# rockcarry/ffcnn

Measured on AMD Instinct MI355X. Metric: frames/sec yolo-fastest-1.1 @320x320 batch-64 per GPU (u8 BGR frames -> net_input's conversion in the first kernel -> full forward: conv stack + YOLO decode + NMS, boxes on rank 0), higher is better.
Workload: dtype f32

## Files before the change

ffcnn_amd/capi.py:

```python
import ctypes as C
import os
import subprocess

import numpy as np

HERE = os.path.dirname(os.path.abspath(__file__))
ROOT = os.path.dirname(HERE)
DATA = os.path.join(ROOT, "data")
CFG = os.path.join(DATA, "yolo-fastest-1.1.cfg")
WEIGHTS = os.path.join(DATA, "yolo-fastest-1.1.weights")

f32p = C.POINTER(C.c_float)


class FFGPU:
    MAX_DET = 128
    MERGE_LDS_SLOTS = 1024
    KEEP_ALL, COMPAT_V6, NO_GRAPH, NO_FUSE, HOST_DETS, SPLIT2, CONCURRENT, BF16_PW = 1, 2, 4, 8, 16, 32, 64, 128
    FEAT_FLAT, FEAT_MEAN, FEAT_MAX = 0, 1, 2
    POST_NONE, POST_SOFTMAX, POST_L2 = 0, 1, 2
    TOPK_MAX = 16
    RELABEL_KEEP_SCORE, RELABEL_LABEL_SCORE = 0, 1
    RELABEL_ENTRIES, RELABEL_MERGED = 0, 1
    K_AUTO, K_GENERIC, K_DW_STREAM, K_DW_LDS, K_PW_MFMA, K_PW_GEMM, _K6, K_DENSE_SMALL, K_IGEMM, K_PW_BF16, K_GROUP_THIN, K_PW_X3, K_CONV_X3, K_PW_X3T = range(14)
# ... 98 lines not shown
class Zone(C.Structure):
    _fields_ = [("x", C.c_float * 8), ("y", C.c_float * 8), ("nverts", C.c_int), ("dwell_frames", C.c_int), ("classes", C.c_uint * 4), ("reserved", C.c_int * 2)]


class Line(C.Structure):
    _fields_ = [("ax", C.c_float), ("ay", C.c_float), ("bx", C.c_float), ("by", C.c_float), ("classes", C.c_uint * 4)]


class Scene(C.Structure):
    _fields_ = [("zone", Zone * 8), ("line", Line * 8), ("nzones", C.c_int), ("nlines", C.c_int), ("anchor", C.c_int), ("reserved", C.c_int)]


class ZonesSpec(C.Structure):
    _fields_ = [("capacity", C.c_int), ("max_missed", C.c_int), ("identity", C.c_int), ("flags", C.c_int), ("min_score", C.c_float),
                ("gate_zone", C.c_uint), ("gate_line", C.c_uint), ("reserved", C.c_int)]


class ZoneSlot(C.Structure):
    _fields_ = [("id", C.c_int), ("px", C.c_float), ("py", C.c_float), ("inside", C.c_int), ("last", C.c_int), ("reserved", C.c_int * 3), ("since", C.c_int * 8)]


class TextItem(C.Structure):
    _fields_ = [("x", C.c_int), ("y", C.c_int), ("fg", C.c_ubyte * 4), ("bg", C.c_ubyte * 4), ("scale", C.c_ubyte), ("flags", C.c_ubyte), ("len", C.c_ubyte),
                ("reserved", C.c_ubyte), ("text", C.c_ubyte * 44)]


class CaptionSpec(C.Structure):
    _fields_ = [("min_score", C.c_float), ("flags", C.c_int), ("identity", C.c_int), ("scale", C.c_int), ("fg", C.c_ubyte * 4), ("color", C.c_ubyte * 4),
                ("palette", C.c_void_p), ("npalette", C.c_int), ("nnames", C.c_int), ("d_names", C.c_void_p)]


class SegItem(C.Structure):
    _fields_ = [("x0", C.c_int), ("y0", C.c_int), ("x1", C.c_int), ("y1", C.c_int), ("color", C.c_ubyte * 4), ("thickness", C.c_ubyte), ("dash", C.c_ubyte),
                ("flags", C.c_ubyte), ("reserved", C.c_ubyte), ("reserved2", C.c_int * 2)]


class OutlineSpec(C.Structure):
    _fields_ = [("flags", C.c_int), ("thickness", C.c_int), ("line_dash", C.c_int), ("marker", C.c_int), ("color", C.c_ubyte * 4), ("alarm", C.c_ubyte * 4),
                ("palette", C.c_void_p), ("npalette", C.c_int), ("reserved", C.c_int)]


class TrailPoint(C.Structure):
    _fields_ = [("x", C.c_int), ("y", C.c_int), ("frame", C.c_int)]


class TrailSlot(C.Structure):
    _fields_ = [("id", C.c_int), ("last", C.c_int), ("n", C.c_int), ("head", C.c_int), ("cx", C.c_int), ("cy", C.c_int), ("reserved", C.c_int * 2),
                ("ring", TrailPoint * 32)]


class TrailsSpec(C.Structure):
    _fields_ = [("capacity", C.c_int), ("max_missed", C.c_int), ("identity", C.c_int), ("flags", C.c_int), ("min_score", C.c_float), ("anchor", C.c_int),
                ("points", C.c_int), ("min_move", C.c_int), ("thickness", C.c_int), ("coast_dash", C.c_int), ("color", C.c_ubyte * 4), ("reserved0", C.c_int),
                ("palette", C.c_void_p), ("npalette", C.c_int), ("reserved", C.c_int)]


class HeatSpec(C.Structure):
    _fields_ = [("gw", C.c_int), ("gh", C.c_int), ("cell_log2", C.c_int), ("mode", C.c_int), ("flags", C.c_int), ("anchor", C.c_int), ("spread", C.c_int),
                ("gain", C.c_int), ("decay_shift", C.c_int), ("min_score", C.c_float), ("classes", C.c_void_p), ("nclasses", C.c_int), ("reserved", C.c_int)]


class HeatBlendSpec(C.Structure):
    _fields_ = [("gw", C.c_int), ("gh", C.c_int), ("cell_log2", C.c_int), ("full_scale", C.c_int), ("floor", C.c_int), ("opacity", C.c_int),
                ("sampling", C.c_int), ("flags", C.c_int), ("palette", C.c_void_p), ("reserved", C.c_int * 2)]


class MotionSpec(C.Structure):
    _fields_ = [("w", C.c_int), ("h", C.c_int), ("cell_log2", C.c_int), ("threshold", C.c_int), ("learn_shift", C.c_int), ("learn_shift_changed", C.c_int),
                ("min_pixels", C.c_int), ("cover", C.c_int), ("warmup", C.c_int), ("flags", C.c_int), ("min_score", C.c_float), ("nclasses", C.c_int),
                ("classes", C.c_void_p), ("reserved", C.c_int * 2)]


MOTION_DETS, MOTION_ROW, MOTION_WORDS, MOTION_MAX_SIDE = 128, 16, 8, 8192
MOTION_GATE_INVERT = 1
MOTION_ENTRIES, MOTION_MERGED = 0, 1
MOTION_ROW_HEADER = ("frame", "changed", "active", "x0", "y0", "x1", "y1", "warm")
MOTION_WORDS_HEADER = ("considered", "dropped", "outside", "moving", "warm", "frames")
MOTION_STATE_HEADER = 16
HEAT_MAX, HEAT_DETS, HEAT_ROW = 2 ** 31 - 1, 128, 8
HEAT_ANCHOR, HEAT_BOX = 0, 1
HEAT_NEAREST, HEAT_SMOOTH = 0, 1
HEAT_RAMP_ALPHA = 1
HEAT_ENTRIES, HEAT_MERGED = 0, 1
HEAT_ROW_HEADER = ("considered", "dropped", "outside", "frame", "peak", "saturated")
HEAT_STATE_HEADER = 16
TRAIL_POINTS, TRAILS_DETS, TRAILS_ROW = 32, 128, 16
TRAILS_COAST, TRAILS_TAPER = 1, 2
TRAILS_ENTRIES, TRAILS_MERGED = 0, 1
TRAILS_ROW_HEADER = ("considered", "known", "fresh", "refused", "duplicate", "anonymous", "dropped", "freed", "live", "frame", "appended", "drawn", "clipped")
TRAILS_STATE_HEADER = 16
SEG_ITEMS, SEG_LIMIT, OUTLINE_FIXED = 512, 1 << 20, 80
OUTLINE_ZONES, OUTLINE_LINES, OUTLINE_TICKS, OUTLINE_MARKERS, OUTLINE_ALARM = 1, 2, 4, 8, 16
TEXT_MAX, TEXT_ITEMS, TEXT_OPAQUE = 44, 256, 1
CAPTION_DETS = 128
CAPTION_NAME, CAPTION_SCORE, CAPTION_ID, CAPTION_OPAQUE = 1, 2, 4, 8
CAPTION_ENTRIES, CAPTION_MERGED = 0, 1
SCENE_ZONES, SCENE_LINES, ZONE_VERTS, ZONES_DETS, ZONES_ROW = 8, 8, 8, 128, 64
ZONES_NONE, ZONES_TYPE, ZONES_IDS = 0, 1, 2
ZONES_GATE_INVERT = 1
ZONES_ENTRIES, ZONES_MERGED = 0, 1
ZONES_EVENTS_HEADER = ("considered", "known", "fresh", "refused", "duplicate", "anonymous", "dropped", "freed", "live", "frame")
ZONES_STATE_HEADER = 144
TRACK_DETS = 128
TRACK_ENTRIES, TRACK_MERGED = 0, 1
TRACK_IDS_HEADER = ("considered", "matched", "born", "refused", "dropped", "freed", "live", "frame")
CROP_F32, CROP_U8 = 0, 1
CROP_ENTRIES, CROP_MERGED = 0, 1
REDACT_FILL, REDACT_MOSAIC = 0, 1
REDACT_OUTSIDE = 1
REDACT_ENTRIES, REDACT_MERGED = 0, 1
BLUR_OUTSIDE = 1
BLUR_ENTRIES, BLUR_MERGED = 0, 1
DRAW_ENTRIES, DRAW_MERGED = 0, 1
YUV_BT601_LIMITED, YUV_BT601_FULL, YUV_BT709_LIMITED, YUV_BT709_FULL = 0, 1, 2, 3

assert C.sizeof(LAYER) == 120 and C.sizeof(NET) == 104 and C.sizeof(BBOX) == 24
assert C.sizeof(FrameDets) == 16 + 24 * FFGPU.MAX_DET
assert C.sizeof(BgrFrame) == 24 and C.sizeof(Nv12Frame) == 40 and C.sizeof(Tile) == 16 and C.sizeof(TileRect) == 16
assert C.sizeof(DrawStyle) == 24 and C.sizeof(CropSpec) == 72 and C.sizeof(Crop) == 48
assert C.sizeof(TrackSpec) == 32 and C.sizeof(Track) == 48
assert C.sizeof(FeatureSpec) == 16 and C.sizeof(Label) == 8 and C.sizeof(RelabelSpec) == 16
assert C.sizeof(Gallery) == 40 and C.sizeof(RedactSpec) == 40 and C.sizeof(BlurSpec) == 40
assert C.sizeof(TextItem) == 64 and C.sizeof(CaptionSpec) == 48
assert C.sizeof(SegItem) == 32 and C.sizeof(OutlineSpec) == 40
assert C.sizeof(TrailPoint) == 12 and C.sizeof(TrailSlot) == 416 and C.sizeof(TrailsSpec) == 64
assert C.sizeof(HeatSpec) == 56 and C.sizeof(HeatBlendSpec) == 48
assert C.sizeof(MotionSpec) == 64
assert C.sizeof(Zone) == 96 and C.sizeof(Line) == 32 and C.sizeof(Scene) == 1040 and C.sizeof(ZonesSpec) == 32 and C.sizeof(ZoneSlot) == 64

BOX_DTYPE = np.dtype([("type", "<i4"), ("score", "<f4"), ("x1", "<f4"), ("y1", "<f4"), ("x2", "<f4"), ("y2", "<f4")])
DETS_DTYPE = np.dtype([("count", "<i4"), ("ncand", "<i4"), ("overflow", "<i4"), ("nfull", "<i4"),
                       ("box", BOX_DTYPE, (FFGPU.MAX_DET,))])
CROP_DTYPE = np.dtype([("target", "<i4"), ("box", "<i4"), ("type", "<i4"), ("score", "<f4"), ("x0", "<i4"), ("y0", "<i4"), ("w", "<i4"), ("h", "<i4"),
                       ("sw", "<i4"), ("sh", "<i4"), ("s1", "<i4"), ("s2", "<i4")])
TRACK_DTYPE = np.dtype([("id", "<i4"), ("type", "<i4"), ("score", "<f4"), ("x1", "<f4"), ("y1", "<f4"), ("x2", "<f4"), ("y2", "<f4"),
                        ("hits", "<i4"), ("missed", "<i4"), ("born", "<i4"), ("det", "<i4"), ("reserved", "<i4")])
ZONE_SLOT_DTYPE = np.dtype([("id", "<i4"), ("px", "<f4"), ("py", "<f4"), ("inside", "<i4"), ("last", "<i4"), ("reserved", "<i4", (3,)), ("since", "<i4", (8,))])
TRAIL_POINT_DTYPE = np.dtype([("x", "<i4"), ("y", "<i4"), ("frame", "<i4")])
TRAIL_SLOT_DTYPE = np.dtype([("id", "<i4"), ("last", "<i4"), ("n", "<i4"), ("head", "<i4"), ("cx", "<i4"), ("cy", "<i4"), ("reserved", "<i4", (2,)),
                             ("ring", TRAIL_POINT_DTYPE, (32,))])
LABEL_DTYPE = np.dtype([("index", "<i4"), ("value", "<f4")])
TEXT_ITEM_DTYPE = np.dtype([("x", "<i4"), ("y", "<i4"), ("fg", "u1", (4,)), ("bg", "u1", (4,)), ("scale", "u1"), ("flags", "u1"), ("len", "u1"), ("reserved", "u1"),
                            ("text", "u1", (44,))])
SEG_ITEM_DTYPE = np.dtype([("x0", "<i4"), ("y0", "<i4"), ("x1", "<i4"), ("y1", "<i4"), ("color", "u1", (4,)), ("thickness", "u1"), ("dash", "u1"), ("flags", "u1"),
                           ("reserved", "u1"), ("reserved2", "<i4", (2,))])

EXPORTS = ["net_load", "net_free", "net_input", "net_forward", "net_dump", "net_profile", "groupconv",
           "ffgpu_device_count", "ffgpu_set_device", "ffgpu_last_error", "ffgpu_build_info",
           "ffgpu_net_weights_dev", "ffgpu_net_weights_commit",
           "ffgpu_exec_create", "ffgpu_exec_destroy", "ffgpu_exec_batch", "ffgpu_exec_arena_bytes",
           "ffgpu_exec_kernel_count", "ffgpu_exec_work_model", "ffgpu_exec_set_scale", "ffgpu_exec_forward_dev", "ffgpu_exec_forward_host",
           "ffgpu_exec_forward_bgr_dev", "ffgpu_exec_forward_bgr_frames_dev", "ffgpu_exec_forward_nv12_frames_dev", "ffgpu_exec_dets_dev", "ffgpu_exec_dets_host", "ffgpu_exec_set_ring", "ffgpu_exec_set_ring_strided", "ffgpu_exec_read_dets", "ffgpu_exec_read_layer", "ffgpu_exec_hash_layers",
           "ffgpu_exec_read_boxes", "ffgpu_exec_cand_capacity", "ffgpu_exec_graph_captures",
           "ffgpu_exec_profile", "ffgpu_exec_profile_steps", "ffgpu_exec_step_model", "ffgpu_groupconv_dev", "ffgpu_groupconv_kernel_name", "ffgpu_groupconv_time_dev", "ffgpu_irb_dev", "ffgpu_irb_plan_text", "ffgpu_irb_stage_plan_text", "ffgpu_front_plan_text", "ffgpu_irb_instantiations", "ffgpu_knobs_text", "ffgpu_dwpw_dev", "ffgpu_packed_records_bytes", "ffgpu_pack_records", "ffgpu_unpack_records",
           "ffgpu_shard_range", "ffgpu_node_create", "ffgpu_node_destroy", "ffgpu_node_ndev", "ffgpu_node_shard", "ffgpu_node_set_scale",
           "ffgpu_node_input_dev", "ffgpu_node_input_slot_dev", "ffgpu_node_depth", "ffgpu_node_rccl_ranks", "ffgpu_node_forward", "ffgpu_node_forward_host",
           "ffgpu_node_submit", "ffgpu_node_wait", "ffgpu_node_run",
           "ffgpu_merge_tiles_scratch_bytes", "ffgpu_merge_tiles_dev", "ffgpu_exec_merge_tiles", "ffgpu_exec_merged_dev", "ffgpu_exec_read_merged",
           "ffgpu_exec_read_merged_boxes", "ffgpu_tile_plan",
           "ffgpu_draw_boxes_bgr_dev", "ffgpu_draw_boxes_nv12_dev", "ffgpu_exec_draw_bgr", "ffgpu_exec_draw_nv12",
           "ffgpu_crop_table_bytes", "ffgpu_crop_slot_bytes", "ffgpu_crop_boxes_bgr_dev", "ffgpu_crop_boxes_nv12_dev", "ffgpu_exec_crop_bgr", "ffgpu_exec_crop_nv12",
           "ffgpu_crops_to_source_dev",
           "ffgpu_track_state_bytes", "ffgpu_track_reset_dev", "ffgpu_track_boxes_dev", "ffgpu_exec_track",
           "ffgpu_feature_dim", "ffgpu_exec_feature_dim", "ffgpu_features_dev", "ffgpu_exec_features", "ffgpu_topk_dev", "ffgpu_crops_relabel_dev",
           "ffgpu_exec_relabel",
           "ffgpu_match_workspace_bytes", "ffgpu_match_dev", "ffgpu_gallery_enroll_dev",
           "ffgpu_redact_boxes_bgr_dev", "ffgpu_redact_boxes_nv12_dev", "ffgpu_exec_redact_bgr", "ffgpu_exec_redact_nv12",
           "ffgpu_blur_boxes_bgr_dev", "ffgpu_blur_boxes_nv12_dev", "ffgpu_exec_blur_bgr", "ffgpu_exec_blur_nv12",
           "ffgpu_zones_state_bytes", "ffgpu_scene_check", "ffgpu_zones_reset_dev", "ffgpu_zones_boxes_dev", "ffgpu_exec_zones",
           "ffgpu_font_builtin", "ffgpu_draw_text_bgr_dev", "ffgpu_draw_text_nv12_dev", "ffgpu_caption_boxes_dev", "ffgpu_exec_caption_bgr", "ffgpu_exec_caption_nv12",
           "ffgpu_caption_scene_dev",
           "ffgpu_draw_segments_bgr_dev", "ffgpu_draw_segments_nv12_dev", "ffgpu_outline_spec_check", "ffgpu_outline_scene_dev",
           "ffgpu_trails_state_bytes", "ffgpu_trails_spec_check", "ffgpu_trails_reset_dev", "ffgpu_trails_boxes_dev", "ffgpu_exec_trails",
           "ffgpu_heat_state_bytes", "ffgpu_heat_spec_check", "ffgpu_heat_blend_spec_check", "ffgpu_heat_palette", "ffgpu_heat_reset_dev", "ffgpu_heat_boxes_dev",
           "ffgpu_exec_heat", "ffgpu_heat_blend_bgr_dev", "ffgpu_heat_blend_nv12_dev",
           "ffgpu_motion_state_bytes", "ffgpu_motion_spec_check", "ffgpu_motion_reset_dev", "ffgpu_motion_update_bgr_dev", "ffgpu_motion_update_nv12_dev",
           "ffgpu_motion_gate_dev", "ffgpu_exec_motion_gate"]
DIAG_EXPORTS = ["ffgpu_membench", "ffgpu_pipe_probe", "ffgpu_pipe_probe2", "ffgpu_pipe_probe3", "ffgpu_mfma_floor", "ffgpu_diag_x3_term", "ffgpu_diag_xl_op", "ffgpu_clock_probe"]


def library_path():
    return os.environ.get("FFCNN_HIP_LIB") or os.path.join(HERE, "lib", "libffcnn_hip.so")


def build_library(force=False):
    cmd = ["make", "-C", os.path.join(HERE, "csrc")]
    if force:
        subprocess.check_call(cmd + ["clean"], stdout=subprocess.DEVNULL)
    subprocess.check_call(cmd, stdout=subprocess.DEVNULL)
    return library_path()


_lib = None


def lib():
    global _lib
    if _lib is not None:
        return _lib
    path = library_path()
    if not os.path.exists(path):
        raise RuntimeError("%s is missing: run `python -c 'import __graft_entry__ as g; g.build()'` "
                           "(the HIP extension is the only compute path)" % path)
    L = C.CDLL(path)
    vp, i, sz = C.c_void_p, C.c_int, C.c_size_t
    L.net_load.restype = C.POINTER(NET)
    L.net_load.argtypes = [C.c_char_p, C.c_char_p, i, i]
    L.net_free.argtypes = [C.POINTER(NET)]
    L.net_input.argtypes = [C.POINTER(NET), vp, i, i, f32p, f32p]
    L.net_forward.argtypes = [C.POINTER(NET)]
    L.net_dump.argtypes = [C.POINTER(NET)]
    L.net_profile.argtypes = [C.POINTER(NET)]
    L.groupconv.argtypes = [f32p, f32p, f32p] + [i] * 12 + [C.POINTER(f32p), C.POINTER(i)]
    L.ffgpu_last_error.restype = C.c_char_p
    L.ffgpu_build_info.restype = C.c_char_p
    if b" DIAG " in L.ffgpu_build_info() and os.environ.get("FFCNN_HIP_ALLOW_DIAG") != "1":
        raise RuntimeError("%s is a DIAG (lab) build of libffcnn_hip; set FFCNN_HIP_ALLOW_DIAG=1 to load it on purpose" % path)
    L.ffgpu_set_device.argtypes = [i]
    L.ffgpu_net_weights_dev.argtypes = [C.POINTER(NET), C.POINTER(vp), C.POINTER(sz)]
    L.ffgpu_net_weights_commit.argtypes = [C.POINTER(NET), vp]
    L.ffgpu_exec_create.restype = vp
    L.ffgpu_exec_create.argtypes = [C.POINTER(NET), i, i]
    L.ffgpu_exec_destroy.argtypes = [vp]
    L.ffgpu_exec_batch.argtypes = [vp]
    L.ffgpu_exec_arena_bytes.restype = sz
    L.ffgpu_exec_arena_bytes.argtypes = [vp]
    L.ffgpu_exec_kernel_count.argtypes = [vp]
    L.ffgpu_exec_work_model.argtypes = [vp, C.POINTER(C.c_double), C.POINTER(C.c_double)]
    L.ffgpu_exec_set_scale.argtypes = [vp, i, i]
    L.ffgpu_exec_forward_dev.argtypes = [vp, vp, vp]
    L.ffgpu_exec_forward_host.argtypes = [vp, f32p]
    L.ffgpu_exec_forward_bgr_dev.argtypes = [vp, vp, i, i, f32p, f32p, vp]
    L.ffgpu_exec_forward_bgr_frames_dev.argtypes = [vp, C.POINTER(BgrFrame), i, f32p, f32p, vp]
    L.ffgpu_exec_forward_nv12_frames_dev.argtypes = [vp, C.POINTER(Nv12Frame), i, f32p, f32p, vp]
    L.ffgpu_exec_dets_dev.argtypes = [vp, C.POINTER(vp), C.POINTER(sz)]
    L.ffgpu_exec_dets_host.restype = vp; L.ffgpu_exec_dets_host.argtypes = [vp]
    L.ffgpu_exec_set_ring.argtypes = [vp, vp, C.c_int]
    L.ffgpu_exec_set_ring_strided.argtypes = [vp, vp, C.c_int, C.c_int]
    L.ffgpu_exec_read_dets.argtypes = [vp, vp, i]
    L.ffgpu_exec_read_layer.argtypes = [vp, i, i, f32p, sz]
    L.ffgpu_exec_hash_layers.argtypes = [vp, vp, i]
    L.ffgpu_exec_profile.argtypes = [vp, vp, f32p]
    L.ffgpu_exec_profile_steps.argtypes = [vp, vp, C.POINTER(i), f32p, i]
    L.ffgpu_exec_step_model.argtypes = [vp, C.POINTER(i), C.POINTER(C.c_double), i]
    L.ffgpu_groupconv_dev.argtypes = [vp, vp, vp] + [i] * 15 + [vp]
    L.ffgpu_groupconv_kernel_name.restype = C.c_char_p
    L.ffgpu_groupconv_kernel_name.argtypes = [i] * 10
    L.ffgpu_groupconv_time_dev.restype = C.c_float
    L.ffgpu_groupconv_time_dev.argtypes = [vp, vp, vp] + [i] * 17 + [vp]
    L.ffgpu_irb_dev.restype = C.c_float
    L.ffgpu_irb_dev.argtypes = [vp] * 6 + [i] * 13 + [vp]
    L.ffgpu_irb_plan_text.argtypes = [i] * 12 + [C.c_char_p, i]
    L.ffgpu_irb_stage_plan_text.argtypes = [i] * 7 + [C.c_char_p, i]
    L.ffgpu_front_plan_text.argtypes = [i] * 4 + [C.c_char_p, i]
    L.ffgpu_irb_instantiations.argtypes = [C.c_char_p, i]
    L.ffgpu_knobs_text.argtypes = [C.c_char_p, i]
    L.ffgpu_exec_read_boxes.argtypes = [vp, i, vp, i]
    L.ffgpu_exec_cand_capacity.argtypes = [vp]
    L.ffgpu_exec_graph_captures.argtypes = [vp]
    L.ffgpu_dwpw_dev.restype = C.c_float
    L.ffgpu_dwpw_dev.argtypes = [vp] * 4 + [i] * 10 + [vp]
    L.ffgpu_packed_records_bytes.restype = C.c_size_t
    L.ffgpu_packed_records_bytes.argtypes = [i, i]
    L.ffgpu_pack_records.restype = i
    L.ffgpu_pack_records.argtypes = [vp, i, C.c_long, i, i, vp, vp]
    L.ffgpu_shard_range.argtypes = [i, i, i, C.POINTER(i), C.POINTER(i)]
    L.ffgpu_shard_range.restype = None
    L.ffgpu_node_create.restype = vp
    L.ffgpu_node_create.argtypes = [C.POINTER(NET), i, C.POINTER(i), i, i, i]
    L.ffgpu_node_destroy.argtypes = [vp]
    L.ffgpu_node_ndev.argtypes = [vp]
    L.ffgpu_node_shard.argtypes = [vp, i, C.POINTER(i), C.POINTER(i), C.POINTER(i)]
    L.ffgpu_node_set_scale.argtypes = [vp, i, i]
    L.ffgpu_node_input_dev.restype = vp
    L.ffgpu_node_input_dev.argtypes = [vp, i]
    L.ffgpu_node_input_slot_dev.restype = vp
    L.ffgpu_node_input_slot_dev.argtypes = [vp, i, i]
    L.ffgpu_node_depth.argtypes = [vp]
    if hasattr(L, "ffgpu_node_rccl_ranks"):
        L.ffgpu_node_rccl_ranks.argtypes = [vp]
    L.ffgpu_node_submit.restype = C.c_long
    L.ffgpu_node_submit.argtypes = [vp, f32p]
    L.ffgpu_node_wait.argtypes = [vp, C.c_long, vp]
    L.ffgpu_node_run.argtypes = [vp, C.c_long, vp]
    L.ffgpu_unpack_records.argtypes = [vp, i, i, vp]
    L.ffgpu_node_forward.argtypes = [vp, vp]
    L.ffgpu_node_forward_host.argtypes = [vp, f32p, vp]
    L.ffgpu_merge_tiles_scratch_bytes.restype = sz
    L.ffgpu_merge_tiles_scratch_bytes.argtypes = [i, i]
    L.ffgpu_merge_tiles_dev.argtypes = [vp, vp, i, C.POINTER(Tile), i, i, C.c_float, i, vp, vp, vp, sz, vp]
    L.ffgpu_exec_merge_tiles.argtypes = [vp, C.POINTER(Tile), i, i, vp]
    L.ffgpu_exec_merged_dev.argtypes = [vp, C.POINTER(vp), C.POINTER(sz)]
    L.ffgpu_exec_read_merged.argtypes = [vp, vp, i]
    L.ffgpu_exec_read_merged_boxes.argtypes = [vp, i, vp, i]
    L.ffgpu_tile_plan.argtypes = [i] * 7 + [C.POINTER(TileRect), i]
    L.ffgpu_draw_boxes_bgr_dev.argtypes = [vp, vp, i, C.POINTER(i), C.POINTER(BgrFrame), i, C.POINTER(DrawStyle), vp]
    L.ffgpu_draw_boxes_nv12_dev.argtypes = [vp, vp, i, C.POINTER(i), C.POINTER(Nv12Frame), i, C.POINTER(DrawStyle), vp]
    L.ffgpu_exec_draw_bgr.argtypes = [vp, i, C.POINTER(BgrFrame), i, C.POINTER(DrawStyle), vp]
    L.ffgpu_exec_draw_nv12.argtypes = [vp, i, C.POINTER(Nv12Frame), i, C.POINTER(DrawStyle), vp]
    L.ffgpu_redact_boxes_bgr_dev.argtypes = [vp, vp, i, C.POINTER(i), C.POINTER(BgrFrame), i, C.POINTER(RedactSpec), vp]
    L.ffgpu_redact_boxes_nv12_dev.argtypes = [vp, vp, i, C.POINTER(i), C.POINTER(Nv12Frame), i, C.POINTER(RedactSpec), vp]
    L.ffgpu_exec_redact_bgr.argtypes = [vp, i, C.POINTER(BgrFrame), i, C.POINTER(RedactSpec), vp]
    L.ffgpu_exec_redact_nv12.argtypes = [vp, i, C.POINTER(Nv12Frame), i, C.POINTER(RedactSpec), vp]
    L.ffgpu_blur_boxes_bgr_dev.argtypes = [vp, vp, i, C.POINTER(i), C.POINTER(BgrFrame), C.POINTER(BgrFrame), i, C.POINTER(BlurSpec), vp]
    L.ffgpu_blur_boxes_nv12_dev.argtypes = [vp, vp, i, C.POINTER(i), C.POINTER(Nv12Frame), C.POINTER(Nv12Frame), i, C.POINTER(BlurSpec), vp]
    L.ffgpu_exec_blur_bgr.argtypes = [vp, i, C.POINTER(BgrFrame), C.POINTER(BgrFrame), i, C.POINTER(BlurSpec), vp]
    L.ffgpu_exec_blur_nv12.argtypes = [vp, i, C.POINTER(Nv12Frame), C.POINTER(Nv12Frame), i, C.POINTER(BlurSpec), vp]
    L.ffgpu_crop_table_bytes.restype = sz
    L.ffgpu_crop_table_bytes.argtypes = [i]
    L.ffgpu_crop_slot_bytes.restype = sz
    L.ffgpu_crop_slot_bytes.argtypes = [i, i, i]
    L.ffgpu_crop_boxes_bgr_dev.argtypes = [vp, vp, i, C.POINTER(i), C.POINTER(BgrFrame), i, C.POINTER(CropSpec), vp, vp, i, vp]
    L.ffgpu_crop_boxes_nv12_dev.argtypes = [vp, vp, i, C.POINTER(i), C.POINTER(Nv12Frame), i, C.POINTER(CropSpec), vp, vp, i, vp]
    L.ffgpu_exec_crop_bgr.argtypes = [vp, i, C.POINTER(BgrFrame), i, C.POINTER(CropSpec), vp, vp, i, vp]
    L.ffgpu_exec_crop_nv12.argtypes = [vp, i, C.POINTER(Nv12Frame), i, C.POINTER(CropSpec), vp, vp, i, vp]
    L.ffgpu_crops_to_source_dev.argtypes = [vp, i, vp, vp, i, vp, vp, vp]
    L.ffgpu_track_state_bytes.restype = sz
    L.ffgpu_track_state_bytes.argtypes = [i, i]
    L.ffgpu_track_reset_dev.argtypes = [vp, i, i, i, vp]
    L.ffgpu_track_boxes_dev.argtypes = [vp, vp, i, C.POINTER(i), C.POINTER(i), i, C.POINTER(TrackSpec), vp, i, vp, vp, vp, vp]
    L.ffgpu_exec_track.argtypes = [vp, i, C.POINTER(i), i, C.POINTER(TrackSpec), vp, i, vp, vp, vp, vp]
    L.ffgpu_zones_state_bytes.restype = sz
    L.ffgpu_zones_state_bytes.argtypes = [i, i]
    L.ffgpu_scene_check.argtypes = [C.POINTER(Scene), i]
    L.ffgpu_zones_reset_dev.argtypes = [vp, i, i, i, vp]
    L.ffgpu_zones_boxes_dev.argtypes = [vp, vp, i, C.POINTER(i), C.POINTER(i), i, C.POINTER(ZonesSpec), vp, vp, i, vp, vp, vp, vp, vp]
    L.ffgpu_exec_zones.argtypes = [vp, i, C.POINTER(i), i, C.POINTER(ZonesSpec), vp, vp, i, vp, vp, vp, vp, vp]
    L.ffgpu_font_builtin.restype = None
    L.ffgpu_font_builtin.argtypes = [vp]
    L.ffgpu_draw_text_bgr_dev.argtypes = [vp, i, vp, C.POINTER(BgrFrame), i, vp]
    L.ffgpu_draw_text_nv12_dev.argtypes = [vp, i, vp, C.POINTER(Nv12Frame), i, vp]
    L.ffgpu_caption_boxes_dev.argtypes = [vp, vp, i, C.POINTER(i), i, C.POINTER(CaptionSpec), vp, vp, i, vp]
    L.ffgpu_exec_caption_bgr.argtypes = [vp, i, C.POINTER(BgrFrame), i, C.POINTER(CaptionSpec), vp, vp, i, vp, vp]
    L.ffgpu_exec_caption_nv12.argtypes = [vp, i, C.POINTER(Nv12Frame), i, C.POINTER(CaptionSpec), vp, vp, i, vp, vp]
    L.ffgpu_caption_scene_dev.argtypes = [vp, vp, i, i, vp, i, C.POINTER(i), i, C.POINTER(CaptionSpec), vp, i, vp]
    L.ffgpu_draw_segments_bgr_dev.argtypes = [vp, i, C.POINTER(BgrFrame), i, vp]
    L.ffgpu_draw_segments_nv12_dev.argtypes = [vp, i, C.POINTER(Nv12Frame), i, vp]
    L.ffgpu_outline_spec_check.argtypes = [C.POINTER(OutlineSpec)]
    L.ffgpu_trails_state_bytes.restype = sz
    L.ffgpu_trails_state_bytes.argtypes = [i, i]
    L.ffgpu_trails_spec_check.argtypes = [C.POINTER(TrailsSpec)]
    L.ffgpu_trails_reset_dev.argtypes = [vp, i, i, i, vp]
    L.ffgpu_trails_boxes_dev.argtypes = [vp, vp, i, C.POINTER(i), C.POINTER(i), i, C.POINTER(TrailsSpec), vp, i, vp, vp, vp, i, i, i, vp]
    L.ffgpu_exec_trails.argtypes = [vp, i, C.POINTER(i), i, C.POINTER(TrailsSpec), vp, i, vp, vp, vp, i, i, i, vp]
    L.ffgpu_heat_state_bytes.restype = sz
    L.ffgpu_heat_state_bytes.argtypes = [i, i, i]
    L.ffgpu_heat_spec_check.argtypes = [C.POINTER(HeatSpec)]
    L.ffgpu_heat_blend_spec_check.argtypes = [C.POINTER(HeatBlendSpec)]
    L.ffgpu_heat_palette.argtypes = [i, vp]
    L.ffgpu_heat_reset_dev.argtypes = [vp, i, i, i, i, vp]
    L.ffgpu_heat_boxes_dev.argtypes = [vp, vp, i, C.POINTER(i), C.POINTER(i), i, C.POINTER(HeatSpec), vp, i, vp, vp]
    L.ffgpu_exec_heat.argtypes = [vp, i, C.POINTER(i), i, C.POINTER(HeatSpec), vp, i, vp, vp]
    L.ffgpu_heat_blend_bgr_dev.argtypes = [vp, i, C.POINTER(i), C.POINTER(BgrFrame), i, C.POINTER(HeatBlendSpec), vp]
    L.ffgpu_heat_blend_nv12_dev.argtypes = [vp, i, C.POINTER(i), C.POINTER(Nv12Frame), i, C.POINTER(HeatBlendSpec), vp]
    L.ffgpu_motion_state_bytes.restype = sz
    L.ffgpu_motion_state_bytes.argtypes = [i, i, i, i]
    L.ffgpu_motion_spec_check.argtypes = [C.POINTER(MotionSpec)]
    L.ffgpu_motion_reset_dev.argtypes = [vp, i, i, i, i, i, vp]
    L.ffgpu_motion_update_bgr_dev.argtypes = [C.POINTER(BgrFrame), i, C.POINTER(i), C.POINTER(MotionSpec), vp, i, vp, vp]
    L.ffgpu_motion_update_nv12_dev.argtypes = [C.POINTER(Nv12Frame), i, C.POINTER(i), C.POINTER(MotionSpec), vp, i, vp, vp]
    L.ffgpu_motion_gate_dev.argtypes = [vp, vp, i, C.POINTER(i), C.POINTER(i), i, C.POINTER(MotionSpec), vp, i, vp, vp, vp, vp]
    L.ffgpu_exec_motion_gate.argtypes = [vp, i, C.POINTER(i), i, C.POINTER(MotionSpec), vp, i, vp, vp, vp, vp]
    L.ffgpu_outline_scene_dev.argtypes = [vp, vp, i, i, vp, i, C.POINTER(i), i, C.POINTER(OutlineSpec), vp, i, vp]
    L.ffgpu_feature_dim.argtypes = [i, i, i, i]
    L.ffgpu_exec_feature_dim.argtypes = [vp, C.POINTER(FeatureSpec)]
    L.ffgpu_features_dev.argtypes = [vp, i, i, i, i, i, i, vp, C.c_long, vp]
    L.ffgpu_exec_features.argtypes = [vp, C.POINTER(FeatureSpec), vp, C.c_long, vp]
    L.ffgpu_topk_dev.argtypes = [vp, i, i, C.c_long, i, vp, vp]
    L.ffgpu_crops_relabel_dev.argtypes = [vp, i, vp, i, vp, vp, i, C.POINTER(i), i, C.POINTER(RelabelSpec), vp, vp, vp]
    L.ffgpu_exec_relabel.argtypes = [vp, i, vp, i, vp, i, i, C.POINTER(RelabelSpec), vp, vp, vp]
    L.ffgpu_match_workspace_bytes.restype = sz
    L.ffgpu_match_workspace_bytes.argtypes = [i, i, i]
    L.ffgpu_match_dev.argtypes = [vp, i, C.c_long, C.POINTER(Gallery), i, vp, vp, C.c_long, vp, sz, vp]
    L.ffgpu_gallery_enroll_dev.argtypes = [C.POINTER(Gallery), vp, i, C.c_long, vp, i, C.c_float, vp, vp]
    _lib = L
    return L


_diag = None


def diag_path():
    return os.path.join(HERE, "lib", "libffcnn_hip_diag.so")


def diag():
    global _diag
    if _diag is None:
        D = C.CDLL(diag_path())
        vp, i, sz = C.c_void_p, C.c_int, C.c_size_t
        D.ffgpu_membench.restype = C.c_float
        D.ffgpu_membench.argtypes = [vp, vp, sz, i, i, i, vp]
        D.ffgpu_pipe_probe.restype = C.c_float
        D.ffgpu_pipe_probe.argtypes = [i, i, i, i, vp]
        D.ffgpu_pipe_probe2.restype = C.c_float
        D.ffgpu_pipe_probe2.argtypes = [i, i, i, i, vp]
        D.ffgpu_pipe_probe3.restype = C.c_float
        D.ffgpu_pipe_probe3.argtypes = [i, i, i, i, i, vp]
        D.ffgpu_clock_probe.argtypes = [C.c_void_p, C.c_int, C.c_int, C.c_void_p]
        D.ffgpu_mfma_floor.restype = C.c_float
        D.ffgpu_mfma_floor.argtypes = [vp, i, i, i, vp]
        _diag = D
    return _diag

# ... 1010 lines not shown
    def submit(self, frames=None):
        if frames is not None:
            frames = np.ascontiguousarray(frames, np.float32)
            assert frames.shape == (self.total,) + self.net.input_shape, frames.shape
        t = lib().ffgpu_node_submit(self.h, frames.ctypes.data_as(f32p) if frames is not None else None)
        if t < 0:
            raise RuntimeError("ffgpu_node_submit failed: %s" % last_error())
        return t

    def wait(self, ticket):
        out = np.zeros(self.total, DETS_DTYPE)
        _check(lib().ffgpu_node_wait(self.h, ticket, out.ctypes.data), "ffgpu_node_wait")
        return out

    def wait_into(self, ticket, out):
        assert out.dtype == DETS_DTYPE and len(out) == self.total and out.flags["C_CONTIGUOUS"]
        _check(lib().ffgpu_node_wait(self.h, ticket, out.ctypes.data), "ffgpu_node_wait")
        return out

    def rccl_ranks(self):
        return lib().ffgpu_node_rccl_ranks(self.h)

    def run(self, steps, out=None):
        if out is None:
            out = np.zeros(self.total, DETS_DTYPE)
        assert out.dtype == DETS_DTYPE and len(out) == self.total and out.flags["C_CONTIGUOUS"]
        _check(lib().ffgpu_node_run(self.h, steps, out.ctypes.data), "ffgpu_node_run")
        return out

    def input_slot_dev(self, rank, slot):
        return lib().ffgpu_node_input_slot_dev(self.h, rank, slot)

    def __init__(self, net, ndev, global_batch, devices=None, exec_flags=0, node_flags=0):
        self.net, self.ndev, self.total = net, ndev, global_batch
        dv = (C.c_int * ndev)(*devices) if devices is not None else None
        self.h = lib().ffgpu_node_create(net.p, ndev, dv, global_batch, exec_flags, node_flags)
        if not self.h:
            raise RuntimeError("ffgpu_node_create failed: %s" % last_error())

    def close(self):
        if self.h:
            lib().ffgpu_node_destroy(self.h)
            self.h = None

    def __enter__(self):
        return self

    def __exit__(self, *a):
        self.close()

    def shard(self, rank):
        lo, hi, dev = C.c_int(), C.c_int(), C.c_int()
        _check(lib().ffgpu_node_shard(self.h, rank, C.byref(lo), C.byref(hi), C.byref(dev)), "ffgpu_node_shard")
        return lo.value, hi.value, dev.value

    def set_scale(self, s1, s2):
        _check(lib().ffgpu_node_set_scale(self.h, s1, s2), "ffgpu_node_set_scale")

    def input_dev(self, rank):
        return lib().ffgpu_node_input_dev(self.h, rank)

    def forward(self):
        out = np.zeros(self.total, DETS_DTYPE)
        _check(lib().ffgpu_node_forward(self.h, out.ctypes.data), "ffgpu_node_forward")
        return out

    def forward_host(self, frames):
        frames = np.ascontiguousarray(frames, np.float32)
        assert frames.shape == (self.total,) + self.net.input_shape, frames.shape
        out = np.zeros(self.total, DETS_DTYPE)
        _check(lib().ffgpu_node_forward_host(self.h, frames.ctypes.data_as(f32p), out.ctypes.data), "ffgpu_node_forward_host")
        return out


def groupconv_dev(d_in, d_filt, d_out, batch, iw, ih, ic, groups, pad, stride, fs, fn, act=0, flags=0, variant=0, stream=None):
    ow, oh = (iw + 2 * pad - fs) // stride + 1, (ih + 2 * pad - fs) // stride + 1
    _check(lib().ffgpu_groupconv_dev(d_in, d_filt, d_out, batch, iw, ih, ic, groups, pad, stride, fs, fn, ow, oh, fn,
                                     act, flags, variant, stream), "ffgpu_groupconv_dev")


def groupconv_time_dev(d_in, d_filt, d_out, batch, iw, ih, ic, groups, pad, stride, fs, fn, act=0, flags=0, variant=0,
                       warmup=5, iters=20, stream=None):
    ow, oh = (iw + 2 * pad - fs) // stride + 1, (ih + 2 * pad - fs) // stride + 1
    us = lib().ffgpu_groupconv_time_dev(d_in, d_filt, d_out, batch, iw, ih, ic, groups, pad, stride, fs, fn, ow, oh, fn,
                                        act, flags, variant, warmup, iters, stream)
    if us < 0:
        raise RuntimeError("ffgpu_groupconv_time_dev failed: %s" % last_error())
    return us


def packed_records_bytes(batch, cap):
    return int(lib().ffgpu_packed_records_bytes(batch, cap))


def pack_records_dev(d_records, nslots, slot_stride_records, batch, cap, d_out, stream=None):
    _check(lib().ffgpu_pack_records(d_records, nslots, slot_stride_records, batch, cap, d_out, stream), "ffgpu_pack_records")


def kernel_name(batch, iw, ih, ic, groups, pad, stride, fs, fn, variant=0):
    return lib().ffgpu_groupconv_kernel_name(batch, iw, ih, ic, groups, pad, stride, fs, fn, variant).decode()


def irb_plan_text(shape, flags=0):
    buf = C.create_string_buffer(1024)
    if lib().ffgpu_irb_plan_text(*shape, flags, buf, len(buf)) < 0:
        raise RuntimeError("ffgpu_irb_plan_text failed: %s" % last_error())
    return buf.value.decode()


def irb_stage_plan_text(batch, iw, ih, blocks, act1=2, actd=2, flags=0):
    buf = C.create_string_buffer(1024)
    if lib().ffgpu_irb_stage_plan_text(batch, iw, ih, blocks, act1, actd, flags, buf, len(buf)) < 0:
        raise RuntimeError("ffgpu_irb_stage_plan_text failed: %s" % last_error())
    return buf.value.decode()


FRONT_FORMS = {"f32": 0, "u8": 1, "bgr_frames": 2, "nv12_frames": 3}


def front_plan_text(batch, pw, ph, form="f32"):
    buf = C.create_string_buffer(256)
    if lib().ffgpu_front_plan_text(batch, pw, ph, FRONT_FORMS[form], buf, len(buf)) < 0:
        raise RuntimeError("ffgpu_front_plan_text failed: %s" % last_error())
    return buf.value.decode()


def irb_instantiations():
    buf = C.create_string_buffer(4096)
    n = lib().ffgpu_irb_instantiations(buf, len(buf))
    if n < 0 or n >= len(buf):
        raise RuntimeError("ffgpu_irb_instantiations failed: %s" % (last_error() if n < 0 else "%d bytes" % n))
    return buf.value.decode().split()


def knobs():
    buf = C.create_string_buffer(1 << 16)
    n = lib().ffgpu_knobs_text(buf, len(buf))
    if n < 0 or n >= len(buf):
        raise RuntimeError("ffgpu_knobs_text failed: %s" % (last_error() if n < 0 else "%d bytes" % n))
    rows = []
    for line in buf.value.decode().splitlines():
        name, kind, dflt, cls, value, text = line.split(" ", 5)
        rows.append({"name": name, "kind": kind, "default": None if dflt == "-" else dflt if dflt == "computed" else int(dflt), "cls": cls, "value": value, "text": text})
    return rows


def dwpw_dev(d_in, d_wd, d_wp, d_out, batch, iw, ih, c, oc, fs, actd=2, actp=0, warmup=0, iters=0, stream=None):
    us = lib().ffgpu_dwpw_dev(d_in, d_wd, d_wp, d_out, batch, iw, ih, c, oc, fs, actd, actp, warmup, iters, stream)
    if us < 0:
        raise RuntimeError("ffgpu_dwpw_dev failed: %s" % last_error())
    return us


def irb_dev(d_in, d_w1, d_wd, d_w2, d_res, d_out, batch, iw, ih, ic, ec, oc, stride, act1=2, actd=2, act2=0, res_act=0,
            warmup=0, iters=0, stream=None):
    us = lib().ffgpu_irb_dev(d_in, d_w1, d_wd, d_w2, d_res, d_out, batch, iw, ih, ic, ec, oc, stride, act1, actd, act2, res_act,
                             warmup, iters, stream)
    if us < 0:
        raise RuntimeError("ffgpu_irb_dev failed: %s" % last_error())
    return us
```

ffcnn_amd/csrc/ffgpu_conv_kernels.inc:

```
#include "ffgpu_dw_stream.inc"
#include "ffgpu_pw_mfma.inc"
#include "ffgpu_pw_gemm32.inc"
#include "ffgpu_pw_bf16.inc"
#include "ffgpu_conv_igemm.inc"
#include "ffgpu_dwpw.inc"
#include "ffgpu_conv_dense.inc"
#include "ffgpu_irb.inc"
#include "ffgpu_irb_thin.inc"
#include "ffgpu_front.inc"
#include "ffgpu_irb_wave.inc"
#include "ffgpu_irb_wave2.inc"
#include "ffgpu_irb_stage.inc"
#include "ffgpu_pw_x3.inc"
#include "ffgpu_pw_x3t.inc"
#include "ffgpu_conv_x3.inc"
#include "ffgpu_dw_lds.inc"
#include "ffgpu_dw_pair.inc"
#include "ffgpu_conv_thin.inc"

struct BareScratch {
    float *p = nullptr; size_t n = 0; int dev = -1;
    float *get(size_t need)
    {
        int d = 0;
// ... 843 lines not shown
    p.ntx = (W + p.TW - 1) / p.TW; p.nty = (H + p.TH - 1) / p.TH;
    p.HW_ = p.TW + fs - 1; p.HH_ = p.TH + fs - 1;
    p.NRT = (p.OC + 15) / 16; p.nchunks = (p.C + 7) / 8;
    int xs = std::max(1, 256 / (8 * p.TH));
    xs = std::min(xs, p.TW);
    int seg = (p.TW + xs - 1) / xs;
    if (seg > 8) { seg = 8; xs = (p.TW + 7) / 8; }
    xs = (p.TW + seg - 1) / seg;
    if (8 * p.TH * xs > 256) return false;
    p.XS = xs; p.SEG = seg;
    p.rld = conv_k4(dw) + 4;
    const int aimg = 2 * p.nchunks * p.NRT * 64 + p.NRT * 32, tapw = fs * fs + 3;
    lds = (size_t)(((aimg + 3) & ~3) + ((p.nchunks * 8 * tapw + 3) & ~3) + ((8 * p.HW_ * p.HH_ + 3) & ~3) + 2 * 8 * p.TPS) * sizeof(float);
    return p.NRT <= 8 && p.NCT <= 8 && lds <= 150 * 1024;
}

bool ffgpu_dwpw_ok(const ConvDesc &dw, const ConvDesc &pw)
{
    DwPwP p; size_t lds;
    return conv_is_depthwise(dw) && (dw.fs == 3 || dw.fs == 5) && dw.stride == 1 && dw.pad == dw.fs / 2 && conv_cnhw_contiguous(dw) && !dw.residual &&
           dw.act != 3 && !(dw.flags & FFGPU_COMPAT_V6) && conv_is_pointwise(pw) && conv_cnhw_contiguous(pw) && !pw.residual && pw.act != 3 &&
           pw.ic == dw.oc && pw.iw == dw.ow && pw.ih == dw.oh && pw.N == dw.N &&
           (long)dw.N * dw.iw * dw.ih * std::max(dw.ic, pw.oc) < (1L << 31) && dwpw_geometry(dw, pw, p, lds);
}

size_t ffgpu_dwpw_pack_floats(const ConvDesc &dw, const ConvDesc &pw)
{
    const int nrt = (pw.oc + 15) / 16, nchunks = (dw.ic + 7) / 8;
    return ((size_t)(2 * nchunks * nrt * 64 + nrt * 32) + 63) & ~(size_t)63;
}

int ffgpu_dwpw_pack(const ConvDesc &dw, const ConvDesc &pw, float *pk, hipStream_t s)
{
    DwPwPackP q;
    q.filt = pw.filt; q.pk = pk; q.C = dw.ic; q.OC = pw.oc; q.NRT = (pw.oc + 15) / 16; q.nchunks = (dw.ic + 7) / 8;
    const int total = 2 * q.nchunks * q.NRT * 64 + q.NRT * 32;
    hipLaunchKernelGGL(k_dwpw_pack, dim3((total + 255) / 256), dim3(256), 0, s, q);
    LAUNCH_OK("dwpw_pack");
    return 0;
}

template <int FS, int SG>
static int dwpw_launch_t(const DwPwP &p, size_t lds, unsigned grid, hipStream_t s)
{
    if (lds_allow((const void *)k_dwpw<FS, SG>, lds, "dwpw")) return -1;
    hipLaunchKernelGGL((k_dwpw<FS, SG>), dim3(grid), dim3(256), lds, s, p);
    LAUNCH_OK("dwpw");
    return 0;
}

int ffgpu_launch_dwpw(const ConvDesc &dw, const ConvDesc &pw, const float *wpack, hipStream_t s)
{
    DwPwP p; size_t lds;
    if (!ffgpu_dwpw_ok(dw, pw) || !dwpw_geometry(dw, pw, p, lds)) { ffgpu_set_error("dwpw: unsupported layer pair"); return -1; }
    p.in = dw.in; p.out = pw.out; p.wd = dw.filt; p.wpack = wpack;
    p.slope_d = dw.act == 2 ? 0.1f : (dw.act == 1 ? 0.f : 1.f); p.slope_p = pw.act == 2 ? 0.1f : (pw.act == 1 ? 0.f : 1.f);
    const unsigned grid = (unsigned)(p.N * p.ntx * p.nty);
    if (dw.fs == 5) return p.SEG <= 4 ? dwpw_launch_t<5, 4>(p, lds, grid, s) : dwpw_launch_t<5, 8>(p, lds, grid, s);
    return p.SEG <= 4 ? dwpw_launch_t<3, 4>(p, lds, grid, s) : dwpw_launch_t<3, 8>(p, lds, grid, s);
}

static float act_slope(int act) { return act == 2 ? 0.1f : (act == 1 ? 0.f : 1.f); }

struct IrbTraceFmt { const char *what; int nd, ns; const char *dname[7], *sname[6]; };
static const IrbTraceFmt irbw_trace = { "irbw", 5, 6, { "issue loads", "barrier", "groups", "reduce", "rows" }, { "expand mfma", "store", "dw0", "prj0", "dw1", "prj1" } };
static const IrbTraceFmt irb_trace = { "irb", 7, 4, { "consts", "wait", "load", "chunks", "reduce", "epilogue", "other-tiles" }, { "bar1", "expand", "bar2", "dw+project" } };
static const IrbTraceFmt &irb_trace_of(const IrbwP &) { return irbw_trace; }
static const IrbTraceFmt &irb_trace_of(const IrbP &) { return irb_trace; }

static unsigned long long *irb_trace_begin(hipStream_t s)
{
    static unsigned long long *d_t = nullptr;
    if (!d_t && hipMalloc(&d_t, 4096 * 16 * sizeof(unsigned long long)) != hipSuccess) return d_t = nullptr;
    (void)hipMemsetAsync(d_t, 0, 4096 * 16 * sizeof(unsigned long long), s);
    return d_t;
}

template <typename P>
static int irb_trace_end(const P &p, const unsigned long long *d_t, long nblocks, hipStream_t s)
{
    const IrbTraceFmt &f = irb_trace_of(p);
    (void)hipStreamSynchronize(s);
    const long nb = std::min(nblocks, 4096L);
    std::vector<unsigned long long> h((size_t)nb * 16);
    (void)hipMemcpy(h.data(), d_t, h.size() * sizeof(unsigned long long), hipMemcpyDeviceToHost);
    unsigned long long t0 = ~0ull, t1 = 0; double d[7] = { 0 }, sum[6] = { 0 }, late = 0;
    for (long b = 0; b < nb; b++) t0 = std::min(t0, h[b * 16]);
    for (long b = 0; b < nb; b++) {
        unsigned long long prev = h[b * 16];
        late = std::max(late, (double)(prev - t0) * 0.01);
        for (int k = 0; k < f.nd; k++) { const unsigned long long t = h[b * 16 + k + 1] ? h[b * 16 + k + 1] : prev; d[k] += (double)(t - prev) / nb * 0.01; prev = t; }
        t1 = std::max(t1, prev);
        for (int k = 0; k < f.ns; k++) sum[k] += (double)h[b * 16 + 8 + k] / nb * 0.01;
    }
    fprintf(stderr, "  trace %s %dx%d %d->%d->%d: span %.2f us (first %ld blocks), last start +%.2f |", f.what, p.W, p.H, p.ic, p.ec, p.oc, (double)(t1 - t0) * 0.01, nb, late);
    for (int k = 0; k < f.nd; k++) fprintf(stderr, " %s %.2f", f.dname[k], d[k]);
    fprintf(stderr, " [");
    for (int k = 0; k < f.ns; k++) fprintf(stderr, "%s%s %.2f", k ? " " : "", f.sname[k], sum[k]);
    fprintf(stderr, "] (us, wave 0, mean per workgroup)\n");
    return 0;
}

template <typename P, void (*K)(P)>
static int irb_launch_t(const P &p, const IrbPlan &c, hipStream_t s)
{
    const char *const what = irb_trace_of(p).what;
    if (lds_allow((const void *)K, (size_t)c.lds, what)) return -1;
    if (knob(K_IRB_TRACE)) {
        P q = p;
        if (!(q.dbg_t = irb_trace_begin(s))) return -1;
        hipLaunchKernelGGL(K, dim3((unsigned)c.grid), dim3(c.block), (size_t)c.lds, s, q);
        return irb_trace_end(p, q.dbg_t, c.grid, s);
    }
    hipLaunchKernelGGL(K, dim3((unsigned)c.grid), dim3(c.block), (size_t)c.lds, s, p);
    LAUNCH_OK(what);
    return 0;
}

#define IRB_LDS_MAX (160 * 1024)

static bool irb_thin_ok(const IrbDesc &d)
{
    return d.stride == 1 && d.ec == 8 && (d.ic == 4 || d.ic == 8) && (d.oc == 4 || d.oc == 8) && d.W % 4 == 0 && d.W / 4 <= 64 &&
           8L * d.N * d.W * d.H < (1L << 30) &&
           d.act1 != 3 && d.actd != 3 && d.act2 != 3 && d.res_act != 3 && !knob(K_NO_THIN);
}

static int thin_band(int N, int H)
{
    int band = 2;
    while (band < 16 && (long)N * H >= 640L * band * 2) band *= 2;
    return band;
}

static ThinP thin_params(const IrbDesc &d)
{
    ThinP p;
    p.in = d.in; p.out = d.out; p.residual = d.residual; p.w1 = d.w1; p.wd = d.wd; p.w2 = d.w2;
    p.W = d.W; p.H = d.H; p.N = d.N;
    p.band = d.plan.band; p.nbands = (d.H + p.band - 1) / p.band;
    p.act1 = act_slope(d.act1); p.actd = act_slope(d.actd); p.act2 = act_slope(d.act2); p.res_act = act_slope(d.res_act);
    p.ntasks = (long)d.N * p.nbands;
    return p;
}

template <int IC, int EC, int OC>
static int irb_thin_launch(const ThinP &p, const IrbPlan &c, hipStream_t s)
{
    hipLaunchKernelGGL((k_irb_thin<IC, EC, OC>), dim3((unsigned)c.grid), dim3(c.block), 0, s, p);
    LAUNCH_OK("irb_thin");
    return 0;
}

typedef int (*IrbThinLaunch)(const ThinP &, const IrbPlan &, hipStream_t);
struct IrbThinKernel { int IC, OC; IrbThinLaunch launch; };
static const IrbThinKernel irb_thin_kernels[] = { { 8, 4, irb_thin_launch<8, 8, 4> }, { 4, 4, irb_thin_launch<4, 8, 4> }, { 8, 8, irb_thin_launch<8, 8, 8> }, { 4, 8, irb_thin_launch<4, 8, 8> } };

static int launch_irb_thin(const IrbDesc &d, hipStream_t s)
{
    const ThinP p = thin_params(d);
    for (const IrbThinKernel &k : irb_thin_kernels)
        if (k.IC == d.ic && k.OC == d.oc) return k.launch(p, d.plan, s);
    ffgpu_set_error("irb_thin: no instantiation for %d -> 8 -> %d channels", d.ic, d.oc);
    return -1;
}

typedef int (*IrbwLaunch)(const IrbwP &, const IrbPlan &, hipStream_t);
struct IrbwKernel { int KS1, OT, S, NSI, NSO; bool big, x3, xl; Knob gate; IrbwLaunch launch; };
#define IRBW_K(ks1, ot, st, nsi, gate) \
    { ks1, ot, st, nsi, 1, true, false, false, gate, irb_launch_t<IrbwP, k_irbw<ks1, ot, st, nsi, true>> }, \
    { ks1, ot, st, nsi, 1, false, false, false, gate, irb_launch_t<IrbwP, k_irbw<ks1, ot, st, nsi, false>> }
static const IrbwKernel irbw_kernels[] = {
    { 2, 1, 1, 3, 2, true, true, false, K_NONE, irb_launch_t<IrbwP, k_irbw2<2, 3, true>> }, { 4, 1, 1, 3, 2, true, true, false, K_NONE, irb_launch_t<IrbwP, k_irbw2<4, 3, true>> },
    { 2, 1, 1, 3, 2, true, false, false, K_NONE, irb_launch_t<IrbwP, k_irbw2<2, 3, false>> }, { 4, 1, 1, 3, 2, true, false, false, K_NONE, irb_launch_t<IrbwP, k_irbw2<4, 3, false>> },
    { 12, 3, 1, 2, 1, true, true, true, K_NONE, irb_launch_t<IrbwP, k_irbw<12, 3, 1, 2, true, true, true>> },
    { 4, 2, 2, 4, 1, true, true, false, K_NONE, irb_launch_t<IrbwP, k_irbw<4, 2, 2, 4, true, true>> },
    { 6, 2, 1, 2, 1, true, true, false, K_NONE, irb_launch_t<IrbwP, k_irbw<6, 2, 1, 2, true, true>> },
    IRBW_K(1, 1, 1, 2, K_NONE), IRBW_K(2, 1, 1, 2, K_NONE), IRBW_K(4, 1, 1, 2, K_NONE), IRBW_K(2, 2, 1, 2, K_NONE), IRBW_K(4, 2, 1, 2, K_NONE),
    IRBW_K(6, 2, 1, 2, K_NONE), IRBW_K(12, 3, 1, 2, K_NONE), IRBW_K(1, 1, 2, 3, K_NONE), IRBW_K(2, 1, 2, 3, K_NONE), IRBW_K(4, 2, 2, 4, K_NONE),
    IRBW_K(6, 3, 2, 3, K_IRBW_S2_633),
    IRBW_K(1, 1, 2, 4, K_IRBW_S2_NSI4), IRBW_K(2, 1, 2, 4, K_IRBW_S2_NSI4),
};
#undef IRBW_K
static const int irbw_nkernels = (int)(sizeof irbw_kernels / sizeof irbw_kernels[0]);

static bool irbw_has_kernel(int KS1, int OT, int S, int NSI)
{
    for (const IrbwKernel &k : irbw_kernels)
        if (k.KS1 == KS1 && k.OT == OT && k.S == S && k.NSI == NSI && k.NSO == 1 && !k.x3) return k.gate == K_NONE || knob(k.gate) != 0;
    return false;
}

static long irbw_ntiles(const IrbDesc &d, int TWq, int TH) { return (long)d.N * ((d.OW + 4 * TWq - 1) / (4 * TWq)) * ((d.OH + TH - 1) / TH); }

static bool irbw_pick(const IrbDesc &d, IrbPlan &c)
{
    if (knob(K_NO_IRBW)) return false;
    if (d.stride != 1 && d.stride != 2) return false;
    if (d.act1 == 3 || d.actd == 3 || d.act2 == 3 || d.res_act == 3) return false;
    if ((size_t)d.ic * d.N * d.H * d.W >= (1u << 30) || (size_t)d.oc * d.N * d.OH * d.OW >= (1u << 30)) return false;
    const int S = d.stride;
    c.KS1 = ((d.ic + 3) & ~3) / 4; c.OT = (d.oc + 15) / 16; c.ngroups = (d.ec + 15) / 16;
    double best = 1e30;
    for (int TWq = 1; TWq <= 8; TWq++) {
        if (TWq > 1 && (TWq - 1) * 4 >= d.OW) break;
        for (int TH = 1; TWq * TH <= 16 && TH <= d.OH + 1; TH++) {
            const int EW = S == 1 ? 4 * TWq + 4 : 8 * TWq + 4, EH = S * (TH - 1) + 3;
            int NSI = (EW * EH + 63) / 64;
            if (NSI < 2) NSI = 2;
            if (S == 2 && NSI < 3) NSI = 3;
            if (NSI > 4 || !irbw_has_kernel(c.KS1, c.OT, S, NSI)) continue;
            const long tiles = irbw_ntiles(d, TWq, TH) / d.N;
            const double cost = (double)tiles * (NSI * (c.KS1 * 128.0 + 500.0) + 4 * (220.0 + c.OT * 128.0)) * (1.0 + 12.0 / EW);
            if (cost < best) { best = cost; c.TWq = TWq; c.TH = TH; c.EW = EW; c.EH = EH; c.NSI = NSI; }
        }
    }
    if (best > 1e29) return false;
    const int ft = knob(K_IRBW_TWQ), fh = knob(K_IRBW_TH);
    if (ft > 0 && fh > 0 && ft * fh <= 16) {
        const int EW = S == 1 ? 4 * ft + 4 : 8 * ft + 4, EH = S * (fh - 1) + 3;
        if (EW * EH <= c.NSI * 64) { c.TWq = ft; c.TH = fh; c.EW = EW; c.EH = EH; }
    }
    const long ntiles = irbw_ntiles(d, c.TWq, c.TH);
    const int regs = c.NSI * c.KS1 * 4 + c.OT * 16 + 2 * (c.KS1 + 4 * c.OT) + 76;
    c.big = regs > 124;
    if (const int f = knob(K_IRBW_BIG); f >= 0) c.big = f != 0;
    if (const int f = S == 2 && c.KS1 == 1 ? knob(K_IRBW_BIG_S2K1) : -1; f >= 0) c.big = f != 0;
    const bool conc = (d.flags & FFGPU_CONCURRENT) != 0;
    const int x3_mask = knob(K_IRBW_X3);
    const int gmax = std::min(8, c.ngroups);
    int G = 1;
    for (int g = 1; g <= gmax; g++) {
        const size_t slot = (size_t)c.OT * 1024, ereg = (size_t)g * 16 * c.NSI * 64;
        if (g > 1 && ereg / slot < (size_t)(g + 1) / 2) continue;
        G = g;
        if (ntiles * g >= knob_or(K_IRBW_GWAVES, conc ? 500 : 1200)) break;
    }
    if (!conc && G > 1 && G < gmax && c.ngroups % G != 0 && (c.ngroups + G) / (G + 1) <= (c.ngroups + G - 1) / G) G++;
    if (d.stride == 1 && c.ngroups == 9 && ntiles >= 400 && ntiles < 512 && gmax >= 4 && !conc && !knob(K_IRBW_NOEXC)) G = 4;
    if (const int f = ntiles >= 256 && ntiles < 1100 ? knob(K_IRBW_G_MID) : 0; f > 0) G = std::min(gmax, f);
    const bool xl_ok = S == 1 && c.KS1 == 12 && c.OT == 3 && c.NSI == 2 && c.big && ((x3_mask >> 3) & 1) != 0;
    if (xl_ok && conc && ntiles < 256) G = std::min(gmax, knob(K_IRBW_G_XL));
    if (const int f = ntiles < 256 ? knob(K_IRBW_G_SMALL) : 0; f > 0) G = std::min(gmax, f);
    const int fg = knob(K_IRBW_G);
    if (fg >= 1 && fg <= gmax) G = fg;
    c.G = G;
    c.NSO = 1;
    c.x3 = S == 1 && c.KS1 == 6 && c.OT == 2 && c.NSI == 2 && c.big && ((x3_mask >> 2) & 1) != 0;
    if (S == 2 && c.KS1 == 4 && c.OT == 2 && c.NSI == 4 && c.big && ((x3_mask >> 4) & 1) != 0) c.x3 = true;
    c.xl = xl_ok && G > 1;
    if (c.xl) c.x3 = true;
    if (G == 1 && S == 1 && c.OT == 1 && (c.KS1 == 2 || c.KS1 == 4) && knob(K_IRBW_NSO) == 2) {
        double best2 = 1e30; int tw2 = 0, th2 = 0;
        for (int TWq = 1; TWq <= 8; TWq++) {
            if (TWq > 1 && (TWq - 1) * 4 >= d.OW) break;
            for (int TH = 1; TWq * TH <= 32 && TH <= d.OH + 1; TH++) {
                if (TWq * TH <= 16 || TWq * ((TH + 1) / 2) > 16) continue;
                const int EW = 4 * TWq + 4, EH = TH + 2;
                if (EW * EH > 192) continue;
                const long tiles = irbw_ntiles(d, TWq, TH) / d.N;
                const double cost = (double)tiles * (3 * (c.KS1 * 128.0 + 500.0) + 2 * 4 * (220.0 + 128.0)) * (1.0 + 12.0 / EW);
                if (cost < best2) { best2 = cost; tw2 = TWq; th2 = TH; }
            }
        }
        const int f2t = knob(K_IRBW2_TWQ), f2h = knob(K_IRBW2_TH);
        if (f2t > 0 && f2h > 0 && f2t * ((f2h + 1) / 2) <= 16 && (4 * f2t + 4) * (f2h + 2) <= 192) { tw2 = f2t; th2 = f2h; best2 = 0; }
        const long nt2 = tw2 ? irbw_ntiles(d, tw2, th2) : 0;
        if (tw2 && best2 < 0.93 * best && nt2 >= knob(K_IRBW2_MIN_TILES)) {
            c.NSO = 2; c.TWq = tw2; c.TH = th2; c.EW = 4 * tw2 + 4; c.EH = th2 + 2; c.NSI = 3; c.big = true; c.WPB = 4; c.xl = false;
            c.x3 = irbw_x3_has(c.KS1) && ((x3_mask >> (c.KS1 == 2 ? 0 : 1)) & 1) != 0;
        }
    }
    {
        const size_t cs = ((size_t)c.ngroups * 224 + c.OT * 32) * sizeof(float), slice = (size_t)16 * c.NSI * 64 * sizeof(float);
        const int cap = c.big ? 12 : 16;
        const int w4 = std::min(cap, (int)(IRB_LDS_MAX / (cs + 4 * slice)) * 4), w8 = std::min(cap, (int)(IRB_LDS_MAX / (cs + 8 * slice)) * 8);
        c.WPB = G > 1 ? G : (w4 >= w8 ? 4 : 8);
        const int fw = knob(K_IRBW_WPB);
        if (G == 1 && fw >= 1 && fw <= 8) c.WPB = fw;
    }
    return true;
}

static void irbw_layout(const IrbPlan &c, int &o_w2, int &o_cs, int &cs_floats, int &total)
{
    o_w2 = c.x3 ? c.ngroups * irbw_x3_nm(c.KS1) * 256 : c.ngroups * c.KS1 * 64;
    o_cs = o_w2 + c.ngroups * 4 * c.OT * 64;
    cs_floats = c.ngroups * 16 * 14 + c.OT * 32;
    total = o_cs + cs_floats;
}

static IrbwP irbw_params(const IrbDesc &d)
{
    const IrbPlan &c = d.plan;
    IrbwP p;
    p.in = d.in; p.out = d.out; p.residual = d.residual; p.pk = d.pk;
    p.N = d.N; p.H = d.H; p.W = d.W; p.OH = d.OH; p.OW = d.OW; p.ic = d.ic; p.ec = d.ec; p.oc = d.oc;
    p.act1 = act_slope(d.act1); p.actd = act_slope(d.actd); p.act2 = act_slope(d.act2); p.res_act = act_slope(d.res_act);
    p.TWq = c.TWq; p.TH = c.TH; p.EW = c.EW; p.EH = c.EH;
    p.tiles_x = (d.OW + 4 * c.TWq - 1) / (4 * c.TWq); p.tiles_y = (d.OH + c.TH - 1) / c.TH;
    p.ntiles = (long)d.N * p.tiles_x * p.tiles_y;
    p.ngroups = c.ngroups; p.G = c.G; p.WPB = c.WPB;
    p.half_last = c.half; p.xcd = c.xcd;
    int total;
    irbw_layout(c, p.o_w2, p.o_cs, p.cs_floats, total);
    p.red_cap = c.region / (c.OT * 1024);
    p.xl_off = p.cs_floats + c.region;
    p.in_elems = (unsigned)((size_t)d.ic * d.N * d.H * d.W);
    p.vec = d.OW % 4 == 0 ? 4 : (d.OW % 2 == 0 ? 2 : 1);
    p.m_ew = (unsigned)(((1ULL << 32) + c.EW - 1) / c.EW);
    p.m_tx = umulhi_magic(p.tiles_x); p.m_ty = umulhi_magic(p.tiles_y); p.m_twq = umulhi_magic(p.TWq);
    p.dbg_t = nullptr;
    return p;
}

static bool irb_plan_wave(IrbDesc &d)
{
// ... 428 lines not shown
```

ffcnn_amd/csrc/ffgpu_dev.hpp:

```cpp
#pragma once
#include <hip/hip_runtime.h>
#include <stddef.h>
#include <stdint.h>
#include <vector>
#include "ffgpu_internal.h"
#include "ffgpu_args.hpp"
#include "ffgpu_streams_host.hpp"
#include "ffgpu_track_host.hpp"
#include "ffgpu_zones_host.hpp"
#include "ffgpu_text_host.hpp"
#include "ffgpu_lines_host.hpp"
#include "ffgpu_trails_host.hpp"
#include "ffgpu_heat_host.hpp"
#include "ffgpu_motion_host.hpp"

#define FFGPU_CHECK(expr)                                                                   \
    do {                                                                                    \
        hipError_t e_ = (expr);                                                             \
        if (e_ != hipSuccess) {                                                             \
            ffgpu_set_error("%s failed: %s (%s:%d)", #expr, hipGetErrorString(e_), __FILE__, __LINE__); \
            return -1;                                                                      \
        }                                                                                   \
    } while (0)

struct ConvDesc {
    const float *in;
    const float *const *in_ind;
    const float *filt;
    float       *out;
    const float *residual;
    const float *wpack;
    int   N;
    int   iw, ih, ic;
    int   ow, oh, oc;
    int   fs, stride, pad, groups;
    int   act;
    int   res_act;
    int   flags;
    long  in_cs, in_ns, out_cs, out_ns, res_cs, res_ns;
    int   nsplit;
    int   kernel;
    int   x3_mt;
};
#define FFGPU_F_BATCH_INPUT (1 << 30)

static inline int conv_k4(const ConvDesc &d) { return (d.fs * d.fs * (d.ic / d.groups) + 3) & ~3; }

enum { IRB_NONE = 0, IRB_THIN, IRB_WAVE, IRB_WG };
struct IrbPlan {
    int family;
    int inst;
    int half;
    int pack_floats;
    int lds, grid, block;
    int KS1, OT, NSI, NSO, TWq, TH, EW, EH, ngroups, G, WPB, big, x3, xl;
    int xcd, region;
    int TW, NF, ECH, NW, KS, wbufs, red_off;
    int band, front_band;
};
struct IrbDesc {
    const float *in; float *out; const float *residual;
    const float *w1, *wd, *w2;
    int N, H, W, OH, OW, ic, ec, oc, stride;
    int act1, actd, act2, res_act;
    const float *pk;
    int flags;
    IrbPlan plan;
};
bool   ffgpu_irb_plan(IrbDesc &d);
size_t ffgpu_irb_pack_floats(const IrbDesc &d);
int    ffgpu_irb_pack(const IrbDesc &d, float *pk, hipStream_t s);
int    ffgpu_launch_irb(const IrbDesc &d, hipStream_t s);
int    ffgpu_irb_plan_line(const IrbDesc &d, char *buf, size_t cap);
int    ffgpu_irb_keys(char *buf, size_t cap);
#define IRBS_MAXB 8
bool   ffgpu_irb_stage_ok(const IrbDesc *blocks, int B);
int    ffgpu_launch_irb_stage(const IrbDesc *blocks, int B, hipStream_t s);
int    ffgpu_irb_stage_line(const IrbDesc *blocks, int B, bool wanted, char *buf, size_t cap);
bool   ffgpu_front_ok(const ConvDesc &c, const IrbDesc &d);
enum InputForm { IN_F32, IN_U8, IN_BGR_FRAMES, IN_NV12_FRAMES, IN_FORMS };
int    ffgpu_launch_front(const ConvDesc &c, const IrbDesc &d, InputForm form, hipStream_t s);
bool   ffgpu_front_nv12_fused();
int    ffgpu_front_plan_line(const IrbDesc &d, InputForm form, char *buf, size_t cap);
int    ffgpu_front_nc(const IrbDesc &d);

bool   ffgpu_dwpw_ok(const ConvDesc &dw, const ConvDesc &pw);
size_t ffgpu_dwpw_pack_floats(const ConvDesc &dw, const ConvDesc &pw);
int    ffgpu_dwpw_pack(const ConvDesc &dw, const ConvDesc &pw, float *pk, hipStream_t s);
int    ffgpu_launch_dwpw(const ConvDesc &dw, const ConvDesc &pw, const float *wpack, hipStream_t s);

size_t ffgpu_pw_pack_floats(const ConvDesc &d);
void   ffgpu_conv_plan(ConvDesc &d);
int    ffgpu_pw_pack(const ConvDesc &d, float *pk, hipStream_t s);

#define FFGPU_YUV_MATRICES { { 16, 298, 409, 100, 208, 516 }, { 0, 256, 359, 88, 183, 454 }, { 16, 298, 459, 55, 136, 541 }, { 0, 256, 403, 48, 120, 475 } }
int  ffgpu_launch_set_frames(FrameDesc *d_tab, const FrameDesc *h_desc, int n, hipStream_t s);
int  ffgpu_launch_input_frames(const FrameDesc *d_tab, bool nv12, float *out, int N, int W, int H, const float mean[3], const float norm[3], hipStream_t s);

struct ExecParams {
    const float *frames;
    int s1, s2;
    ffgpu_frame_dets *ring;
    int ring_slots, ring_stride;
    int bbox_max;
    const unsigned char *bgr;
    long  bgr_frame;
    int   bgr_pitch;
    float mean[3], norm[3];
    const FrameDesc *frames_tab;
};
int  ffgpu_launch_set_params(ExecParams *d_prm, const ExecParams &v, hipStream_t s);
bool ffgpu_conv_supports_ind(const ConvDesc &d);

bool ffgpu_no_device(const char *what);

int         ffgpu_launch_conv(const ConvDesc &d, int variant, hipStream_t s);
const char *ffgpu_conv_kernel_name(const ConvDesc &d, int variant);
int ffgpu_launch_pool(const float *in, float *out, int N, int c, int w, int h, int fs, int stride, int is_max, hipStream_t s);
int ffgpu_launch_spp(const float *in, float *const out[3], const int fs[3], int n, long planes, int w, int h, hipStream_t s);
int ffgpu_launch_upsample(const float *in, float *out, long planes, int w, int h, int stride, hipStream_t s);
int ffgpu_launch_add_act(const float *a, const float *b, float *out, long n, int act, hipStream_t s);
int ffgpu_launch_copy(const float *src, float *dst, long n, hipStream_t s);
int ffgpu_launch_hash64(const float *x, long n, unsigned long long *out, hipStream_t s);
int ffgpu_launch_input_bgr(const unsigned char *bgr, float *out, int N, int w, int h, int W, int H,
                           int sw, int sh, int s1, int s2, const float mean[3], const float norm[3], hipStream_t s);

struct YoloHead {
    const float *in;
    int   w, h, classes;
    int   anchors[3][2];
    float thresh, scale_xy;
    int   key_base;
};
int ffgpu_launch_yolo(const YoloHead &hd, int N, int netw, int neth, BBOX *cand, int *cand_key, int *ncand, int cap, int *ring_ctr, hipStream_t s);
int ffgpu_launch_nms(const BBOX *cand, const int *cand_key, int *ncand, int cap, BBOX *full, void *scratch,
                     ffgpu_frame_dets *dets, ffgpu_frame_dets *dets_host, const int *ring_ctr, int N,
                     float thresh, int use_min, const ExecParams *prm, hipStream_t s);
#define FFGPU_NMS_LDS_CAP 8192
bool ffgpu_nms_in_lds(int cap_pow2);
int ffgpu_launch_clear(int *ncand, int N, int *ring_ctr, hipStream_t s);

int    ffgpu_merge_build_tab(const char *what, const ffgpu_tile *tiles, int ntiles, int nimages, std::vector<int> &tab, std::vector<int> *off);
size_t ffgpu_merge_tab_bytes(int ntiles);
int    ffgpu_launch_set_ints(int *d_dst, const int *h_src, int n, hipStream_t s);
int    ffgpu_launch_merge_tiles(const int *d_tab, const std::vector<int> &tab, const ffgpu_frame_dets *recs, const BBOX *lists, int stride,
                                float thresh, int use_min, ffgpu_frame_dets *out_recs, BBOX *out_lists, void *scratch, hipStream_t s);

int ffgpu_draw_style_check(const char *what, const ffgpu_draw_style *st, unsigned pal[256], int *npal);
int ffgpu_launch_draw(bool nv12, const DetSource &src, const std::vector<DrawTarget> &targets, const unsigned pal[256], int npal, int thickness, hipStream_t s);

struct CropPlan {
    int   out_w, out_h, form, per_target, nclasses, num, den;
    float min_score, mean[3], norm[3];
    unsigned char classes[256];
};
int ffgpu_box_sel_check(const char *what, int nclasses, const unsigned char *classes, int margin_num, int margin_den);
int ffgpu_crop_spec_check(const char *what, const ffgpu_crop_spec *sp, CropPlan &pl);
int ffgpu_crop_buffers_check(const char *what, const void *d_out, const void *d_table, int capacity);
int ffgpu_launch_crop(bool nv12, const DetSource &src, const std::vector<CropSrc> &sources, const CropPlan &pl, void *d_out, void *d_table, int capacity, hipStream_t s);

struct RedactPlan {
    int   mode, cell, outside, nclasses, num, den;
    float min_score;
    unsigned colour;
    unsigned char classes[256];
};
int ffgpu_redact_spec_check(const char *what, const ffgpu_redact_spec *sp, bool nv12, RedactPlan &pl);
int ffgpu_launch_redact(const char *what, bool nv12, const DetSource &src, const std::vector<DrawTarget> &targets, const RedactPlan &pl, hipStream_t s);

struct BlurPlan {
    int   radius, passes, outside, nclasses, num, den;
    float min_score;
    unsigned char classes[256];
};
int ffgpu_blur_spec_check(const char *what, const ffgpu_blur_spec *sp, BlurPlan &pl);
int ffgpu_launch_blur(const char *what, bool nv12, const DetSource &src, const std::vector<DrawTarget> &targets, const std::vector<DrawTarget> &scratch,
                      const BlurPlan &pl, hipStream_t s);

int ffgpu_state_reset(const char *what, void *d_state, size_t all, int nstreams, int which_stream, void *stream);

int ffgpu_launch_track(const DetSource &src, const int *streams, int ntargets, const ffgpu_track_spec &spec, void *d_state, void *d_ids, void *d_out_records, void *d_out_lists, hipStream_t s);

int ffgpu_launch_zones(const DetSource &src, const int *streams, int ntargets, const ffgpu_zones_spec &spec, const void *d_scenes, void *d_state, const void *d_ids,
                       void *d_events, void *d_out_records, void *d_out_lists, hipStream_t s);

int ffgpu_launch_draw_text(bool nv12, const void *d_items, int items_stride, const void *d_font, const std::vector<DrawTarget> &targets, hipStream_t s);
int ffgpu_launch_caption_boxes(const DetSource &src, int ntargets, const CaptionPlan &pl, const void *d_ids, void *d_items, int items_stride, hipStream_t s);

int ffgpu_launch_draw_segments(bool nv12, const void *d_items, int items_stride, const std::vector<DrawTarget> &targets, hipStream_t s);

int ffgpu_launch_trails(const DetSource &src, const int *streams, int ntargets, const TrailsPlan &pl, void *d_state, const void *d_ids, void *d_rows, void *d_items,
                        int items_stride, int first_item, int nitems, hipStream_t s);

int ffgpu_launch_heat(const DetSource &src, const int *streams, int ntargets, const HeatPlan &pl, void *d_state, void *d_rows, hipStream_t s);

int ffgpu_launch_motion_gate(const DetSource &src, const int *streams, int ntargets, const MotionPlan &pl, const void *d_state, void *d_words, void *d_out_records,
                             void *d_out_lists, hipStream_t s);

int ffgpu_feature_args_check(const char *what, int n, int c, int h, int w, int pool, int post, const void *d_out, long out_stride);
int ffgpu_launch_features(const float *const *parts, int nparts, int pn, int c, int h, int w, int pool, int post, float *d_out, long out_stride, hipStream_t s);
int ffgpu_relabel_args_check(const char *what, const void *d_table, int capacity, const void *d_labels, int k, int ntargets, const ffgpu_relabel_spec *spec,
                             const void *d_out_records);
int ffgpu_launch_relabel(const void *d_table, int capacity, const void *d_labels, int k, const DetSource &src, int ntargets, const ffgpu_relabel_spec &spec,
                         void *d_out_records, void *d_out_lists, hipStream_t s);
```

ffcnn_amd/csrc/ffgpu_exec.hip:

```cpp
#include <algorithm>
#include <cstdarg>
#include <cstdint>
#include <cstdio>
#include <cstdlib>
#include <cstring>
#include <map>
#include <mutex>
#include <string>
#include <type_traits>
#include <vector>

#include "ffgpu_dev.hpp"
#include "ffgpu_knobs.hpp"
#include "ffgpu_plan.hpp"
#include "conv.h"

static thread_local char g_err[512] = "";

extern "C" void ffgpu_set_error(const char *fmt, ...)
{
    va_list ap;
    va_start(ap, fmt);
    vsnprintf(g_err, sizeof g_err, fmt, ap);
    va_end(ap);
// ... 1664 lines not shown
        if (copy_h2d(ex->d_input, net->layer_list[0].data, sizeof(float) * (size_t)ex->in_c * ex->in_h * ex->in_w)) return -1;
        float us[LAYER_TYPE_TOTOAL];
        if (ffgpu_exec_profile(ex, ex->d_input, us)) return -1;
        for (int k = 0; k < LAYER_TYPE_TOTOAL; k++) { dev->us_acc[k] += us[k]; net->timeused[k] = (int)(dev->us_acc[k] / 1000.0 + 0.5); }
    } else if (ffgpu_exec_forward_host(ex, net->layer_list[0].data)) return -1;
    static thread_local ffgpu_frame_dets rec;
    if (ffgpu_exec_read_dets(ex, &rec, 1) != 1) return -1;
    const ffcnn_ext *ext = ffcnn_ext_of(net);
    const int nb = std::max(0, std::min(rec.nfull, std::min(net->bbox_max, ext ? ext->box_cap : FFGPU_MAX_DET)));
    if (nb <= FFGPU_MAX_DET) memcpy(net->bbox_list, rec.box, sizeof(BBOX) * (size_t)nb);
    else if (ffgpu_exec_read_boxes(ex, 0, net->bbox_list, nb) < 0) return -1;
    net->bbox_num = nb;
    return 0;
}

extern "C" int ffgpu_netdev_profile_us(void *p, double us_by_kind[LAYER_TYPE_TOTOAL])
{
    ffgpu_netdev *dev = (ffgpu_netdev *)p;
    if (!dev) return -1;
    for (int k = 0; k < LAYER_TYPE_TOTOAL; k++) us_by_kind[k] = dev->us_acc[k];
    return 0;
}

extern "C" int ffgpu_net_weights_dev(NET *net, void **dev_ptr, size_t *bytes)
{
    ffgpu_netdev *dev = netdev_of(net);
    if (!dev) return -1;
    if (dev_ptr) *dev_ptr = dev->d_weights;
    if (bytes) *bytes = sizeof(float) * (size_t)net->weight_size;
    return 0;
}

extern "C" int ffgpu_net_weights_commit(NET *net, void *stream)
{
    ffgpu_netdev *dev = netdev_of(net);
    if (!dev) return -1;
    std::lock_guard<std::mutex> lk(dev->mu);
    for (ffgpu_exec *ex : dev->execs)
        if (repack(ex, stream ? (hipStream_t)stream : ex->own_stream)) return -1;
    if (!stream) for (ffgpu_exec *ex : dev->execs) FFGPU_CHECK(hipStreamSynchronize(ex->own_stream));
    return 0;
}

#include "ffgpu_node.inc"

static void fill_desc(ConvDesc &d, const float *in, const float *filt, float *out, int batch,
                      int iw, int ih, int ic, int groups, int pad, int stride, int fs, int ow, int oh, int oc, int act, int flags)
{
    memset(&d, 0, sizeof d);
    d.in = in; d.filt = filt; d.out = out; d.N = batch;
    d.iw = iw; d.ih = ih; d.ic = ic; d.ow = ow; d.oh = oh; d.oc = oc;
    d.fs = fs; d.stride = stride; d.pad = pad; d.groups = groups; d.act = act; d.flags = flags & (FFGPU_COMPAT_V6 | FFGPU_BF16_PW);
    d.in_cs = (long)batch * iw * ih; d.in_ns = (long)iw * ih;
    d.out_cs = (long)batch * ow * oh; d.out_ns = (long)ow * oh;
}

extern "C" int ffgpu_groupconv_dev(const float *d_in, const float *d_filt, float *d_out, int batch,
                                   int iw, int ih, int ic, int groups, int pad, int stride,
                                   int fs, int fn, int ow, int oh, int oc, int act,
                                   int flags, int variant, void *stream)
{
    if (!d_in || !d_filt || !d_out || batch < 1 || fn != oc) { ffgpu_set_error("groupconv_dev: bad arguments"); return -1; }
    ConvDesc d;
    fill_desc(d, d_in, d_filt, d_out, batch, iw, ih, ic, groups, pad, stride, fs, ow, oh, oc, act, flags);
    return ffgpu_launch_conv(d, variant, (hipStream_t)stream);
}

extern "C" const char *ffgpu_groupconv_kernel_name(int batch, int iw, int ih, int ic, int groups, int pad,
                                                   int stride, int fs, int fn, int variant)
{
    ConvDesc d;
    const int ow = (iw + 2 * pad - fs) / stride + 1, oh = (ih + 2 * pad - fs) / stride + 1;
    fill_desc(d, nullptr, nullptr, nullptr, batch, iw, ih, ic, groups, pad, stride, fs, ow, oh, fn, 0, 0);
    return ffgpu_conv_kernel_name(d, variant);
}

extern "C" float ffgpu_groupconv_time_dev(const float *d_in, const float *d_filt, float *d_out, int batch,
                                          int iw, int ih, int ic, int groups, int pad, int stride,
                                          int fs, int fn, int ow, int oh, int oc, int act,
                                          int flags, int variant, int warmup, int iters, void *stream)
{
    if (iters < 1 || fn != oc) { ffgpu_set_error("groupconv_time_dev: bad arguments"); return -1.f; }
    hipStream_t s = (hipStream_t)stream;
    ConvDesc d;
    fill_desc(d, d_in, d_filt, d_out, batch, iw, ih, ic, groups, pad, stride, fs, ow, oh, oc, act, flags);
    float *pk = nullptr;
    if (variant == FFGPU_K_AUTO && ffgpu_pw_pack_floats(d) > 0) {
        if (hipMalloc(&pk, ffgpu_pw_pack_floats(d) * sizeof(float)) != hipSuccess || ffgpu_pw_pack(d, pk, s)) { ffgpu_set_error("pack failed"); return -1.f; }
        d.wpack = pk;
    }
    hipEvent_t e0, e1;
    if (hipEventCreate(&e0) != hipSuccess || hipEventCreate(&e1) != hipSuccess) { ffgpu_set_error("hipEventCreate failed"); return -1.f; }
    for (int i = 0; i < warmup; i++) if (ffgpu_launch_conv(d, variant, s)) return -1.f;
    (void)hipEventRecord(e0, s);
    for (int i = 0; i < iters; i++) if (ffgpu_launch_conv(d, variant, s)) return -1.f;
    (void)hipEventRecord(e1, s);
    if (hipEventSynchronize(e1) != hipSuccess) { ffgpu_set_error("hipEventSynchronize: %s", hipGetErrorString(hipGetLastError())); return -1.f; }
    float ms = 0.f;
    (void)hipEventElapsedTime(&ms, e0, e1);
    (void)hipEventDestroy(e0); (void)hipEventDestroy(e1);
    return ms * 1000.f / iters;
}

static void irb_fill(IrbDesc &d, int batch, int iw, int ih, int ic, int ec, int oc, int stride, int act1, int actd, int act2, int res_act)
{
    d.N = batch; d.H = ih; d.W = iw; d.OH = (ih + 2 - 3) / stride + 1; d.OW = (iw + 2 - 3) / stride + 1;
    d.ic = ic; d.ec = ec; d.oc = oc; d.stride = stride;
    d.act1 = act1; d.actd = actd; d.act2 = act2; d.res_act = res_act;
}

extern "C" int ffgpu_irb_plan_text(int batch, int iw, int ih, int ic, int ec, int oc, int stride, int act1, int actd, int act2, int res_act, int flags, char *buf, int cap)
{
    if (!buf || cap < 1 || batch < 1 || iw < 1 || ih < 1 || stride < 1) { ffgpu_set_error("irb_plan_text: bad arguments"); return -1; }
    IrbDesc d{};
    irb_fill(d, batch, iw, ih, ic, ec, oc, stride, act1, actd, act2, res_act);
    d.flags = flags & FFGPU_CONCURRENT;
    (void)ffgpu_irb_plan(d);
    return ffgpu_irb_plan_line(d, buf, (size_t)cap);
}

extern "C" int ffgpu_front_plan_text(int batch, int pw, int ph, int form, char *buf, int cap)
{
    if (!buf || cap < 1 || batch < 1 || pw < 1 || ph < 1 || form < 0 || form >= IN_FORMS) { ffgpu_set_error("front_plan_text: bad arguments"); return -1; }
    IrbDesc d{};
    irb_fill(d, batch, pw, ph, 8, 8, 4, 1, 0, 0, 0, 0);
    if (!ffgpu_irb_plan(d) || d.plan.family != IRB_THIN) return snprintf(buf, (size_t)cap, "unsupported");
    return ffgpu_front_plan_line(d, (InputForm)form, buf, (size_t)cap);
}

extern "C" int ffgpu_irb_stage_plan_text(int batch, int iw, int ih, int blocks, int act1, int actd, int flags, char *buf, int cap)
{
    if (!buf || cap < 1 || batch < 1 || iw < 1 || ih < 1 || blocks < 1 || blocks > 64) { ffgpu_set_error("irb_stage_plan_text: bad arguments"); return -1; }
    std::vector<IrbDesc> run((size_t)blocks, IrbDesc{});
    for (IrbDesc &d : run) {
        irb_fill(d, batch, iw, ih, 48, 224, 48, 1, act1, actd, 0, 0);
        d.flags = flags & FFGPU_CONCURRENT;
        if (!ffgpu_irb_plan(d)) return snprintf(buf, (size_t)cap, "unsupported");
    }
    return ffgpu_irb_stage_line(run.data(), blocks, stage_wanted(batch, flags), buf, (size_t)cap);
}

extern "C" int ffgpu_irb_instantiations(char *buf, int cap)
{
    if (!buf || cap < 1) { ffgpu_set_error("irb_instantiations: bad arguments"); return -1; }
    return ffgpu_irb_keys(buf, (size_t)cap);
}

extern "C" int ffgpu_knobs_text(char *buf, int cap)
{
    if (!buf || cap < 1) { ffgpu_set_error("knobs_text: bad arguments"); return -1; }
    return ffgpu_knobs_lines(buf, (size_t)cap);
}

extern "C" float ffgpu_irb_dev(const float *d_in, const float *d_w1, const float *d_wd, const float *d_w2,
                               const float *d_res, float *d_out, int batch, int iw, int ih, int ic, int ec, int oc,
                               int stride, int act1, int actd, int act2, int res_act, int warmup, int iters, void *stream)
{
    hipStream_t s = (hipStream_t)stream;
    IrbDesc d{};
    d.in = d_in; d.out = d_out; d.residual = d_res; d.w1 = d_w1; d.wd = d_wd; d.w2 = d_w2;
    irb_fill(d, batch, iw, ih, ic, ec, oc, stride, act1, actd, act2, res_act);
    if (!d_in || !d_out || !d_w1 || !d_wd || !d_w2 || !ffgpu_irb_plan(d)) { ffgpu_set_error("irb_dev: unsupported block shape"); return -1.f; }
    float *pk = nullptr;
    if (hipMalloc(&pk, ffgpu_irb_pack_floats(d) * sizeof(float)) != hipSuccess) { ffgpu_set_error("irb_dev: hipMalloc failed"); return -1.f; }
    d.pk = pk;
    float us = 0.f;
    int rc = ffgpu_irb_pack(d, pk, s);
    if (!rc && iters <= 0) rc = ffgpu_launch_irb(d, s);
    if (!rc && iters > 0) {
        hipEvent_t e0, e1;
        (void)hipEventCreate(&e0); (void)hipEventCreate(&e1);
        for (int i = 0; i < warmup && !rc; i++) rc = ffgpu_launch_irb(d, s);
        (void)hipEventRecord(e0, s);
        for (int i = 0; i < iters && !rc; i++) rc = ffgpu_launch_irb(d, s);
        (void)hipEventRecord(e1, s);
        (void)hipEventSynchronize(e1);
        float ms = 0.f;
        (void)hipEventElapsedTime(&ms, e0, e1);
        us = ms * 1000.f / iters;
        (void)hipEventDestroy(e0); (void)hipEventDestroy(e1);
    }
    (void)hipStreamSynchronize(s);
    (void)hipFree(pk);
    return rc ? -1.f : us;
}

extern "C" float ffgpu_dwpw_dev(const float *d_in, const float *d_wd, const float *d_wp, float *d_out, int batch, int iw, int ih,
                                int c, int oc, int fs, int actd, int actp, int warmup, int iters, void *stream)
{
    hipStream_t s = (hipStream_t)stream;
    ConvDesc dw, pw;
    fill_desc(dw, d_in, d_wd, nullptr, batch, iw, ih, c, c, fs / 2, 1, fs, iw, ih, c, actd, 0);
    fill_desc(pw, nullptr, d_wp, d_out, batch, iw, ih, c, 1, 0, 1, 1, iw, ih, oc, actp, 0);
    if (!d_in || !d_wd || !d_wp || !d_out || !ffgpu_dwpw_ok(dw, pw)) { ffgpu_set_error("dwpw_dev: unsupported layer pair"); return -1.f; }
    float *pk = nullptr;
    if (hipMalloc(&pk, ffgpu_dwpw_pack_floats(dw, pw) * sizeof(float)) != hipSuccess) { ffgpu_set_error("dwpw_dev: hipMalloc failed"); return -1.f; }
    float us = 0.f;
    int rc = ffgpu_dwpw_pack(dw, pw, pk, s);
    if (!rc && iters <= 0) rc = ffgpu_launch_dwpw(dw, pw, pk, s);
    if (!rc && iters > 0) {
        hipEvent_t e0, e1;
        (void)hipEventCreate(&e0); (void)hipEventCreate(&e1);
        for (int i = 0; i < warmup && !rc; i++) rc = ffgpu_launch_dwpw(dw, pw, pk, s);
        (void)hipEventRecord(e0, s);
        for (int i = 0; i < iters && !rc; i++) rc = ffgpu_launch_dwpw(dw, pw, pk, s);
        (void)hipEventRecord(e1, s);
        (void)hipEventSynchronize(e1);
        float ms = 0.f;
        (void)hipEventElapsedTime(&ms, e0, e1);
        us = ms * 1000.f / iters;
        (void)hipEventDestroy(e0); (void)hipEventDestroy(e1);
    }
    (void)hipStreamSynchronize(s);
    (void)hipFree(pk);
    return rc ? -1.f : us;
}

struct HostConvScratch { float *in = nullptr, *filt = nullptr, *out = nullptr; size_t in_n = 0, filt_n = 0, out_n = 0; int dev = -1; };

static int grow(float **p, size_t *have, size_t need)
{
    if (*have >= need) return 0;
    (void)hipFree(*p);
    *p = nullptr; *have = 0;
    FFGPU_CHECK(hipMalloc(p, need * sizeof(float)));
    *have = need;
    return 0;
}

extern "C" void groupconv(float *in, float *filt, float *out,
                          int iw, int ih, int ic, int ig, int ipad, int istride,
                          int fs, int fn, int ow, int oh, int oc, int act,
                          float **scratch, int *scratch_floats)
{
    static thread_local HostConvScratch sc;
    (void)scratch; (void)scratch_floats;
    if (!in || !filt || !out || ig < 1 || ic % ig) { fprintf(stderr, "ffcnn groupconv: bad arguments\n"); return; }
    const size_t n_in = (size_t)iw * ih * ic, n_out = (size_t)ow * oh * oc;
    const size_t n_f = (size_t)fn * ((((size_t)fs * fs * (ic / ig) + 3) & ~(size_t)3) + 4);
    const int flags = knob(K_COMPAT_V6) ? FFGPU_COMPAT_V6 : 0;
    int cur = 0;
    (void)hipGetDevice(&cur);
    if (sc.dev != cur) {
        (void)hipFree(sc.in); (void)hipFree(sc.filt); (void)hipFree(sc.out);
        sc = HostConvScratch();
        sc.dev = cur;
    }
    int rc = grow(&sc.in, &sc.in_n, n_in) || grow(&sc.filt, &sc.filt_n, n_f) || grow(&sc.out, &sc.out_n, n_out);
    if (!rc) rc = copy_h2d(sc.in, in, n_in * sizeof(float)) || copy_h2d(sc.filt, filt, n_f * sizeof(float));
    if (!rc) rc = ffgpu_groupconv_dev(sc.in, sc.filt, sc.out, 1, iw, ih, ic, ig, ipad, istride, fs, fn, ow, oh, oc, act, flags, FFGPU_K_AUTO, nullptr);
    if (!rc) rc = hipStreamSynchronize(nullptr) != hipSuccess || copy_d2h(out, sc.out, n_out * sizeof(float));
    if (rc) fprintf(stderr, "ffcnn groupconv: device path failed: %s\n", g_err[0] ? g_err : hipGetErrorString(hipGetLastError()));
}
```

ffcnn_amd/csrc/ffgpu_irb_thin.inc:

```
struct ThinP {
    const float *in; float *out; const float *residual;
    const float *w1, *wd, *w2;
    int W, H, N;
    int band, nbands;
    float act1, actd, act2, res_act;
    long ntasks;
};

typedef float v2f_t __attribute__((ext_vector_type(2)));

template <int IC, int EC, int OC>
__global__ void __launch_bounds__(256) __attribute__((amdgpu_waves_per_eu(2))) k_irb_thin(ThinP p)
{
    static_assert(EC % 2 == 0 && OC % 2 == 0, "channel pairs");
    constexpr int K4 = (IC + 3) & ~3, RL1 = K4 + 4, RL2 = ((EC + 3) & ~3) + 4, OCP = (OC + 3) & ~3, CP = EC / 2;
    constexpr int T1 = (IC + 2) * 2, TD = 24, T2 = 2 * OCP;
    __shared__ __attribute__((aligned(16))) float tw[CP * (T1 + TD + T2) + 2 * OCP];
    float *t1 = tw, *td = tw + CP * T1, *t2 = td + CP * TD, *tsb = t2 + CP * T2;
    for (int i = threadIdx.x; i < CP * T1; i += 256) {
        const int cp = i / T1, j = (i % T1) >> 1, c = 2 * cp + (i & 1);
        t1[i] = p.w1[c * RL1 + (j < IC ? j : K4 + (j - IC))];
    }
    for (int i = threadIdx.x; i < CP * TD; i += 256) {
        const int cp = i / TD, j = (i % TD) >> 1, c = 2 * cp + (i & 1);
        td[i] = j < 9 ? p.wd[c * 16 + j] : (j < 11 ? p.wd[c * 16 + 3 + j] : 0.f);
    }
    for (int i = threadIdx.x; i < CP * T2; i += 256) {
        const int cp = i / T2, h = (i % T2) / OCP, k = i % OCP;
        t2[i] = k < OC ? p.w2[k * RL2 + 2 * cp + h] : 0.f;
    }
    for (int i = threadIdx.x; i < 2 * OCP; i += 256) { const int k = i % OCP; tsb[i] = k < OC ? p.w2[k * RL2 + RL2 - 4 + i / OCP] : 0.f; }
    __syncthreads();
    const int lane = threadIdx.x & 63;
    const int task = blockIdx.x * 4 + __builtin_amdgcn_readfirstlane(threadIdx.x >> 6);
    if (task >= p.ntasks) return;
    const int n = task / p.nbands, band_i = task - n * p.nbands;
    const int lpr = p.W >> 2;
    const bool on = lane < lpr, last_col = lane == lpr - 1;
    const long HW = (long)p.W * p.H;
    const unsigned cs = (unsigned)p.N * (unsigned)HW;
    const unsigned lo = on ? lane * 4 : 0;
    const float *ip = p.in + (long)n * HW;
    float *op = p.out + (long)n * HW;
    const float *rp = p.residual ? p.residual + (long)n * HW : nullptr;
    const int y0 = band_i * p.band, y1 = min(y0 + p.band, p.H);
    const v2f_t z2 = { 0.f, 0.f };

    auto load_row = [&](int r, v4f (&x)[IC]) {
        const unsigned ro = (unsigned)min(max(r, 0), p.H - 1) * p.W + lo;
#pragma unroll
        for (int ci = 0; ci < IC; ci++) x[ci] = *reinterpret_cast<const v4f *>(ip + (ci * cs + ro));
    };
    struct W1T { v4f q[T1 / 4]; };
    struct WDT { v4f q[TD / 4]; v4f w2[T2 / 4]; };
    auto ld1 = [&](int cp) { W1T r;
#pragma unroll
        for (int j = 0; j < T1 / 4; j++) r.q[j] = *reinterpret_cast<const v4f *>(t1 + cp * T1 + 4 * j);
        return r; };
    auto ldd = [&](int cp) { WDT r;
#pragma unroll
        for (int j = 0; j < TD / 4; j++) r.q[j] = *reinterpret_cast<const v4f *>(td + cp * TD + 4 * j);
#pragma unroll
        for (int j = 0; j < T2 / 4; j++) r.w2[j] = *reinterpret_cast<const v4f *>(t2 + cp * T2 + 4 * j);
        return r; };
    auto pairof = [](const v4f (&q)[TD / 4 > T1 / 4 ? TD / 4 : T1 / 4], int j) { return (j & 1) ? (v2f_t){ q[j >> 1].z, q[j >> 1].w } : (v2f_t){ q[j >> 1].x, q[j >> 1].y }; };
    (void)pairof;

    v2f_t A[2][CP][4];
    v4f X[2][IC];
#pragma unroll
    for (int c = 0; c < CP; c++)
#pragma unroll
        for (int j = 0; j < 4; j++) A[0][c][j] = A[1][c][j] = z2;
    load_row(y0 - 1, X[0]);

    auto step = [&](int r, auto PAR) {
        constexpr int P = decltype(PAR)::value;
        asm volatile("" ::: "memory");
        const bool rin = r >= 0 && r < p.H, fin = r > y0;
        const v4f (&x)[IC] = X[P];
        v4f res[OC];
        if (r < y1) load_row(r + 1, X[P ^ 1]);
        if (fin && rp) {
#pragma unroll
            for (int k = 0; k < OC; k++) res[k] = *reinterpret_cast<const v4f *>(rp + (k * cs + (unsigned)(r - 1) * p.W + lo));
        }
        v2f_t o[OCP / 2][4];
#pragma unroll
        for (int k = 0; k < OCP / 2; k++)
#pragma unroll
            for (int j = 0; j < 4; j++) o[k][j] = z2;
        W1T n1 = ld1(0);
        __builtin_amdgcn_sched_barrier(0);
#pragma unroll
        for (int cp = 0; cp < CP; cp++) {
            const W1T c1 = n1;
            const WDT cd = ldd(cp);
            __builtin_amdgcn_sched_barrier(0);
            auto w1p = [&](int j) { return (j & 1) ? (v2f_t){ c1.q[j >> 1].z, c1.q[j >> 1].w } : (v2f_t){ c1.q[j >> 1].x, c1.q[j >> 1].y }; };
            auto wdp = [&](int j) { return (j & 1) ? (v2f_t){ cd.q[j >> 1].z, cd.q[j >> 1].w } : (v2f_t){ cd.q[j >> 1].x, cd.q[j >> 1].y }; };
            v2f_t win[6];
            if (rin) {
#pragma unroll
                for (int j = 0; j < 4; j++) {
                    v2f_t a = w1p(0) * x[0][j];
#pragma unroll
                    for (int ci = 1; ci < IC; ci++) a += w1p(ci) * x[ci][j];
                    a = a * w1p(IC) + w1p(IC + 1);
                    const v2f_t u = a * p.act1;
                    win[1 + j] = (v2f_t){ act_max(a.x, u.x, act_floor(p.act1)), act_max(a.y, u.y, act_floor(p.act1)) };
                }
            } else {
#pragma unroll
                for (int j = 0; j < 4; j++) win[1 + j] = z2;
            }
            if (cp + 1 < CP) n1 = ld1(cp + 1);
            win[0] = (v2f_t){ dpp_shr1(win[4].x), dpp_shr1(win[4].y) };
            const v2f_t sr = { dpp_shl1(win[1].x), dpp_shl1(win[1].y) };
            win[5] = (v2f_t){ last_col ? 0.f : sr.x, last_col ? 0.f : sr.y };
            __builtin_amdgcn_sched_barrier(0);
            if (fin) {
#pragma unroll
                for (int j = 0; j < 4; j++) {
                    v2f_t d = A[P][cp][j];
                    d += wdp(6) * win[j]; d += wdp(7) * win[j + 1]; d += wdp(8) * win[j + 2];
                    d = d * wdp(9) + wdp(10);
                    const v2f_t u = d * p.actd;
                    d = (v2f_t){ act_max(d.x, u.x, act_floor(p.actd)), act_max(d.y, u.y, act_floor(p.actd)) };
#pragma unroll
                    for (int k = 0; k < OCP / 2; k++) {
                        const v4f &wa = cd.w2[k >> 1], &wb = cd.w2[(OCP / 2 + k) >> 1];
                        const v2f_t w2a = (k & 1) ? (v2f_t){ wa.z, wa.w } : (v2f_t){ wa.x, wa.y };
                        const v2f_t w2b = ((OCP / 2 + k) & 1) ? (v2f_t){ wb.z, wb.w } : (v2f_t){ wb.x, wb.y };
                        o[k][j] += w2a * d.x;
                        o[k][j] += w2b * d.y;
                    }
                }
            }
#pragma unroll
            for (int j = 0; j < 4; j++) {
                v2f_t m = A[P ^ 1][cp][j];
                m += wdp(3) * win[j]; m += wdp(4) * win[j + 1]; m += wdp(5) * win[j + 2];
                A[P ^ 1][cp][j] = m;
                v2f_t s = wdp(0) * win[j];
                s += wdp(1) * win[j + 1]; s += wdp(2) * win[j + 2];
                A[P][cp][j] = s;
            }
#pragma unroll
            for (int j = 0; j < 4; j++) asm volatile("" : "+v"(A[0][cp][j]), "+v"(A[1][cp][j]));
            if (fin) {
#pragma unroll
                for (int k = 0; k < OCP / 2; k++)
#pragma unroll
                    for (int j = 0; j < 4; j++) asm volatile("" : "+v"(o[k][j]));
            }
            __builtin_amdgcn_sched_barrier(0);
        }
        if (fin && on) {
            v4f sb[2 * OCP / 4];
#pragma unroll
            for (int j = 0; j < 2 * OCP / 4; j++) sb[j] = *reinterpret_cast<const v4f *>(tsb + 4 * j);
#pragma unroll
            for (int k = 0; k < OC / 2; k++) {
                const v4f &sq = sb[k >> 1], &bq = sb[(OCP / 2 + k) >> 1];
                const v2f_t sc = (k & 1) ? (v2f_t){ sq.z, sq.w } : (v2f_t){ sq.x, sq.y };
                const v2f_t bi = ((OCP / 2 + k) & 1) ? (v2f_t){ bq.z, bq.w } : (v2f_t){ bq.x, bq.y };
                v2f_t v[4];
#pragma unroll
                for (int j = 0; j < 4; j++) {
                    const v2f_t t = o[k][j] * sc + bi, u = t * p.act2;
                    v[j] = (v2f_t){ act_max(t.x, u.x, act_floor(p.act2)), act_max(t.y, u.y, act_floor(p.act2)) };
                }
#pragma unroll
                for (int h = 0; h < 2; h++) {
                    v4f q = { v[0][h], v[1][h], v[2][h], v[3][h] };
                    if (rp) {
                        q += res[2 * k + h];
                        q.x = act_max(q.x, p.res_act * q.x, act_floor(p.res_act)); q.y = act_max(q.y, p.res_act * q.y, act_floor(p.res_act)); q.z = act_max(q.z, p.res_act * q.z, act_floor(p.res_act)); q.w = act_max(q.w, p.res_act * q.w, act_floor(p.res_act));
                    }
                    *reinterpret_cast<v4f *>(op + ((2 * k + h) * cs + (unsigned)(r - 1) * p.W + lo)) = q;
                }
            }
        }
    };
    int r = y0 - 1;
    for (; r < y1; r += 2) {
        step(r, std::integral_constant<int, 0>());
        step(r + 1, std::integral_constant<int, 1>());
    }
    if (r == y1) step(r, std::integral_constant<int, 0>());
}
```

ffcnn_amd/csrc/ffgpu_knobs.hpp:

```cpp
#pragma once
#include <assert.h>
#include <limits.h>
#include <stdio.h>
#include <stdlib.h>

enum KnobKind { KNOB_INT, KNOB_ON, KNOB_SET, KNOB_TEXT };
enum KnobClass { KNOB_PRODUCT, KNOB_TUNING, KNOB_TEST, KNOB_LAB };
#define KNOB_COMPUTED INT_MIN

#define FFGPU_KNOBS_MAIN(X) \
     \
    X(COMPAT_V6,         "FFCNN_COMPAT_V6",         ON,   0,             PRODUCT, "the reference's v6 behaviour for 5x5 filters (executors and groupconv)") \
    X(NO_GRAPH,          "FFGPU_NO_GRAPH",          ON,   0,             PRODUCT, "eager launches instead of a captured graph (as the flag FFGPU_NO_GRAPH)") \
    X(BF16_PW,           "FFGPU_BF16_PW",           ON,   0,             PRODUCT, "opt-in bf16 inputs for compute-bound pointwise layers; own tolerance (as the flag)") \
    X(NO_FUSE,           "FFGPU_NO_FUSE",           ON,   0,             PRODUCT, "one kernel per layer: no fused blocks, no concat in place, no residual in the conv epilogue (as the flag)") \
    X(BRANCH,            "FFGPU_BRANCH",            ON,   0,             PRODUCT, "first detection head as a parallel graph branch instead of in line") \
    X(DWPW,              "FFGPU_DWPW",              ON,   0,             PRODUCT, "the heads' depthwise + pointwise pairs as one kernel (measured slower)") \
    X(NO_U8_FRONT,       "FFGPU_NO_U8_FRONT",       SET,  0,             PRODUCT, "u8 frames through the staging kernel and the fp32 first kernel even where they could go straight in") \
    X(NV12_FRONT,        "FFGPU_NV12_FRONT",        INT,  KNOB_COMPUTED, PRODUCT, "1: NV12 frames into the NV12 form of k_front where the plan has it, 0: staged; default: the build's measured choice") \
    X(VERBOSE,           "FFGPU_VERBOSE",           SET,  0,             PRODUCT, "print every error to stderr as it is set") \
    X(NODE_PACK_BOXES,   "FFGPU_NODE_PACK_BOXES",   INT,  0,             PRODUCT, "room per frame in a shard's packed record block; 0 or less: 16, the constant of the same name in ffgpu_node.inc") \
    X(NO_IRB,            "FFGPU_NO_IRB",            ON,   0,             TUNING,  "no fused inverted-residual blocks: their three layers as three kernels") \
    X(IRB_MIN_EC,        "FFGPU_IRB_MIN_EC",        INT,  24,            TUNING,  "fewest expanded channels of a block the planner fuses (thin blocks apart)") \
    X(IRB_STAGE,         "FFGPU_IRB_STAGE",         INT,  1,             TUNING,  "runs of 48 -> 224 -> 48 blocks on a small plane as one launch in FFGPU_CONCURRENT executors of 32 frames or more (0: one launch per block)") \
    X(SPLIT_PARTS,       "FFGPU_SPLIT_PARTS",       INT,  2,             TUNING,  "parallel chains of an FFGPU_SPLIT2 executor: 2, 4 or 8 (where the batch divides)") \
    X(NO_INDIRECT,       "FFGPU_NO_INDIRECT",       ON,   0,             TEST,    "the first kernel takes the input address from its arguments, not the parameter block: graphs keyed by input pointer") \
     \
    X(FORCE_GENERIC,     "FFGPU_FORCE_GENERIC",     INT,  0,             PRODUCT, "the reference-order generic kernel for every convolution") \
    X(PW_X3,             "FFGPU_PW_X3",             INT,  1,             PRODUCT, "0: never pick the split-bf16 pointwise kernel k_pw_x3") \
    X(PWX3_MIN_IC,       "FFGPU_PWX3_MIN_IC",       INT,  192,           TUNING,  "k_pw_x3: fewest input channels AUTO takes it for") \
    X(PWX3_MIN_OC,       "FFGPU_PWX3_MIN_OC",       INT,  256,           TUNING,  "k_pw_x3: fewest output channels") \
    X(PWX3_MIN_P,        "FFGPU_PWX3_MIN_P",        INT,  65536,         TUNING,  "k_pw_x3: fewest pixels") \
    X(PWX3_MT,           "FFGPU_PWX3_MT",           INT,  0,             TUNING,  "k_pw_x3: 16-row blocks per wave, 1 / 2 / 4 (0: 4)") \
    X(PW_X3T,            "FFGPU_PW_X3T",            INT,  1,             PRODUCT, "0: never pick the tiled split-bf16 GEMM k_pw_x3t") \
    X(PWX3T_MIN_IC,      "FFGPU_PWX3T_MIN_IC",      INT,  128,           TUNING,  "k_pw_x3t: fewest input channels AUTO takes it for") \
    X(PWX3T_MIN_OC,      "FFGPU_PWX3T_MIN_OC",      INT,  192,           TUNING,  "k_pw_x3t: fewest output channels") \
    X(PWX3T_MIN_P,       "FFGPU_PWX3T_MIN_P",       INT,  65536,         TUNING,  "k_pw_x3t: fewest pixels") \
    X(PWXT_TM,           "FFGPU_PWXT_TM",           INT,  256,           TUNING,  "k_pw_x3t: channels per workgroup tile, 256 or 128 (frozen with a plan: ConvDesc::x3_mt)") \
    X(PWXT_NARROW,       "FFGPU_PWXT_NARROW",       INT,  1,             TUNING,  "k_pw_x3t: 0 switches the narrow tiles of the partial last round off") \
    X(PWXT_PERSIST,      "FFGPU_PWXT_PERSIST",      INT,  0,             TUNING,  "k_pw_x3t: persistent workgroups over the main tiles") \
    X(PWXT_NT,           "FFGPU_PWXT_NT",           INT,  -1,            TUNING,  "k_pw_x3t: non-temporal output stores never (0) / always (1); -1: outputs of 128 MB and more") \
    X(PWXT_DBG,          "FFGPU_PWXT_DBG",          INT,  0,             LAB,     "k_pw_x3t: ablation mask handed to the kernel (wrong results)") \
    X(PW_X3S,            "FFGPU_PW_X3S",            INT,  1,             PRODUCT, "0: never pick the pointwise form of k_conv_x3 (pw_x3s)") \
    X(PWX3S_MIN_IC,      "FFGPU_PWX3S_MIN_IC",      INT,  96,            TUNING,  "pw_x3s: fewest input channels AUTO takes it for") \
    X(PWX3S_MIN_OC,      "FFGPU_PWX3S_MIN_OC",      INT,  64,            TUNING,  "pw_x3s: fewest output channels") \
    X(PWX3S_MIN_WGS,     "FFGPU_PWX3S_MIN_WGS",     INT,  64,            TUNING,  "pw_x3s: fewest workgroups") \
    X(IG_X3,             "FFGPU_IG_X3",             INT,  1,             PRODUCT, "0: never pick the split-bf16 dense 3x3 kernel k_conv_x3") \
    X(IGX3_S2,           "FFGPU_IGX3_S2",           INT,  1,             TUNING,  "k_conv_x3: 0 keeps the stride-2 layers on the fp32 implicit GEMM") \
    X(IGX3_NW,           "FFGPU_IGX3_NW",           INT,  0,             TUNING,  "k_conv_x3: waves per workgroup, 4 or 8 (0: 8 at stride 2, else 4)") \
    X(IGX3_MT,           "FFGPU_IGX3_MT",           INT,  0,             TUNING,  "k_conv_x3: 16-row blocks per wave, 1 / 2 / 4 (0: by shape; frozen with a plan: ConvDesc::x3_mt)") \
    X(IGX3_MT4_WGS,      "FFGPU_IGX3_MT4_WGS",      INT,  192,           TUNING,  "k_conv_x3: fewest workgroups that four blocks per wave must leave") \
    X(IGX3_MIN_IC,       "FFGPU_IGX3_MIN_IC",       INT,  16,            TUNING,  "k_conv_x3: fewest input channels AUTO takes it for") \
    X(IGX3_MIN_WGS,      "FFGPU_IGX3_MIN_WGS",      INT,  160,           TUNING,  "k_conv_x3: fewest workgroups AUTO takes it for") \
    X(PWG_MIN_OC,        "FFGPU_PWG_MIN_OC",        INT,  128,           TUNING,  "k_pw_gemm32: fewest output channels AUTO takes it for") \
    X(PWG_MIN_IC,        "FFGPU_PWG_MIN_IC",        INT,  64,            TUNING,  "k_pw_gemm32: fewest input channels") \
    X(NO_PW_GEMM,        "FFGPU_NO_PW_GEMM",        INT,  0,             PRODUCT, "never pick k_pw_gemm32: k_pw_mfma instead") \
    X(NO_IGEMM,          "FFGPU_NO_IGEMM",          INT,  0,             TUNING,  "never pick the implicit GEMMs (k_conv_igemm, the dense form of k_conv_x3)") \
    X(NO_GROUP_THIN,     "FFGPU_NO_GROUP_THIN",     INT,  0,             TUNING,  "never pick k_conv_thin for grouped layers of few channels per group") \
    X(NO_DW_PAIR,        "FFGPU_NO_DW_PAIR",        INT,  0,             PRODUCT, "depthwise layers on k_dw_lds instead of k_dw_pair") \
    X(NO_CONV_FIRST,     "FFGPU_NO_CONV_FIRST",     INT,  0,             PRODUCT, "the first layer on the dense small-channel kernel instead of k_conv_first") \
    X(CONV_FIRST_MIN_PX, "FFGPU_CONV_FIRST_MIN_PX", INT,  262144,        TUNING,  "k_conv_first: fewest output pixels of the batch") \
    X(NO_POOL2X2,        "FFGPU_NO_POOL2X2",        INT,  0,             TEST,    "2x2 / stride 2 max pooling on the general pool kernel") \
     \
    X(IGEMM_NOVEC,       "FFGPU_IGEMM_NOVEC",       INT,  0,             TUNING,  "k_conv_igemm: no vector form of the gather") \
    X(IGEMM_SPLIT,       "FFGPU_IGEMM_SPLIT",       INT,  0,             TUNING,  "k_conv_igemm: split-K factor 1 .. 16 (0: by tile count; frozen with a plan: ConvDesc::nsplit)") \
    X(DW_U,              "FFGPU_DW_U",              INT,  4,             TUNING,  "k_dw3_stream: rows per step, 1 / 2 / 4") \
    X(DW_BAND,           "FFGPU_DW_BAND",           INT,  4,             TUNING,  "k_dw3_stream: rows per wave task (0: enough tasks to fill the chip)") \
    X(DW_NT,             "FFGPU_DW_NT",             INT,  -1,            PRODUCT, "k_dw3_stream: stream past the caches never (0) / always (1); -1: outputs of 128 MB and more") \
    X(DW_XCD,            "FFGPU_DW_XCD",            INT,  0,             TUNING,  "k_dw3_stream: walk the tasks XCD by XCD") \
    X(DWP_NI,            "FFGPU_DWP_NI",            INT,  0,             TUNING,  "k_dw_pair: frames per workgroup, at most (0: by shape)") \
    X(DWL_BH,            "FFGPU_DWL_BH",            INT,  0,             TUNING,  "k_dw_lds: rows per band (0: by shape)") \
    X(DWL_NPL,           "FFGPU_DWL_NPL",           INT,  0,             TUNING,  "k_dw_lds: planes per item (0: by shape)") \
    X(PWG_WM,            "FFGPU_PWG_WM",            INT,  0,             TUNING,  "k_pw_gemm32: waves per workgroup, 4 or 8 (0: 8 from 248 output channels; part of the packed image)") \
    X(PWG_NARROW,        "FFGPU_PWG_NARROW",        INT,  1,             TUNING,  "k_pw_gemm32: 0 switches the narrow tiles of the partial last round off") \
    X(PWG_DBG,           "FFGPU_PWG_DBG",           INT,  0,             LAB,     "k_pw_gemm32: ablation mask handed to the kernel (wrong results)") \
     \
    X(NO_THIN,           "FFGPU_NO_THIN",           INT,  0,             PRODUCT, "8-channel blocks on the wave kernel instead of k_irb_thin") \
    X(THIN_BAND,         "FFGPU_THIN_BAND",         INT,  KNOB_COMPUTED, TUNING,  "k_irb_thin: rows per wave; default by batch and height (thin_band)") \
    X(FRONT_BAND,        "FFGPU_FRONT_BAND",        INT,  KNOB_COMPUTED, TUNING,  "k_front: rows per wave; default as FFGPU_THIN_BAND") \
    X(NO_FRONT,          "FFGPU_NO_FRONT",          INT,  0,             PRODUCT, "layers 0-3 as k_conv_first + k_irb_thin instead of k_front") \
    X(FRONT_MIN_PX,      "FFGPU_FRONT_MIN_PX",      INT,  262144,        TUNING,  "k_front: fewest output pixels of the batch") \
    X(FRONT_NC,          "FFGPU_FRONT_NC",          INT,  3,             PRODUCT, "k_front: output columns per lane, 3 where a row fits a wave that way, or 4") \
    X(NO_IRBW,           "FFGPU_NO_IRBW",           INT,  0,             PRODUCT, "fused blocks on the workgroup kernel k_irb instead of the wave-autonomous k_irbw") \
    X(IRBW_S2_633,       "FFGPU_IRBW_S2_633",       INT,  1,             TUNING,  "k_irbw: 0 hides the stride-2 form for 24 input / 48 output channels from the planner") \
    X(IRBW_S2_NSI4,      "FFGPU_IRBW_S2_NSI4",      INT,  0,             TUNING,  "k_irbw: 1 lets the planner take the four-strip halo for the thin stride-2 blocks") \
    X(IRBW_TWQ,          "FFGPU_IRBW_TWQ",          INT,  0,             TUNING,  "k_irbw: tile width in quads (with FFGPU_IRBW_TH; 0: searched)") \
    X(IRBW_TH,           "FFGPU_IRBW_TH",           INT,  0,             TUNING,  "k_irbw: tile height (with FFGPU_IRBW_TWQ; 0: searched)") \
    X(IRBW_BIG,          "FFGPU_IRBW_BIG",          INT,  -1,            TUNING,  "k_irbw: the 256-register form never (0) / always (1); -1: by register need") \
    X(IRBW_BIG_S2K1,     "FFGPU_IRBW_BIG_S2K1",     INT,  -1,            TUNING,  "k_irbw: as FFGPU_IRBW_BIG for the stride-2 blocks of at most 4 input channels alone") \
    X(IRBW_GWAVES,       "FFGPU_IRBW_GWAVES",       INT,  KNOB_COMPUTED, TUNING,  "k_irbw: waves a launch wants before the group split stops; default 1200, 500 with FFGPU_CONCURRENT") \
    X(IRBW_NOEXC,        "FFGPU_IRBW_NOEXC",        INT,  0,             TUNING,  "k_irbw: without the measured exception (four waves on the 20x20 blocks)") \
    X(IRBW_G_MID,        "FFGPU_IRBW_G_MID",        INT,  0,             TUNING,  "k_irbw: group split for 256 .. 1099 tiles (0: as computed)") \
    X(IRBW_X3,           "FFGPU_IRBW_X3",           INT,  30,            PRODUCT, "fused blocks: expand GEMM as split-bf16 products, one bit per shape: 0: 8 input channels, 1: 16, 2: 24, 3: 48 (split tile in LDS), 4: the 40 -> 20 stride-2 block") \
    X(IRBW_G_XL,         "FFGPU_IRBW_G_XL",         INT,  7,             TUNING,  "k_irbw: group split of the LDS-resident form with several chains in flight") \
    X(IRBW_G_SMALL,      "FFGPU_IRBW_G_SMALL",      INT,  0,             TUNING,  "k_irbw: group split under 256 tiles (0: as computed)") \
    X(IRBW_G,            "FFGPU_IRBW_G",            INT,  0,             TUNING,  "k_irbw: group split, wins over everything (0: as computed)") \
    X(IRBW_NSO,          "FFGPU_IRBW_NSO",          INT,  2,             TUNING,  "k_irbw2: anything but 2 keeps the planner off the two-strip kernel") \
    X(IRBW2_TWQ,         "FFGPU_IRBW2_TWQ",         INT,  0,             TUNING,  "k_irbw2: tile width in quads (with FFGPU_IRBW2_TH; 0: searched)") \
    X(IRBW2_TH,          "FFGPU_IRBW2_TH",          INT,  0,             TUNING,  "k_irbw2: tile height (with FFGPU_IRBW2_TWQ; 0: searched)") \
    X(IRBW2_MIN_TILES,   "FFGPU_IRBW2_MIN_TILES",   INT,  768,           TUNING,  "k_irbw2: fewest tiles the planner takes it for") \
    X(IRBW_WPB,          "FFGPU_IRBW_WPB",          INT,  0,             TUNING,  "k_irbw: tiles per workgroup without a group split, 1 .. 8 (0: 4 or 8 by LDS)") \
    X(IRBW_HALF,         "FFGPU_IRBW_HALF",         INT,  1,             PRODUCT, "0: a last group of at most 8 real expanded channels is computed as a whole group") \
    X(IRBW_XCD,          "FFGPU_IRBW_XCD",          INT,  3,             PRODUCT, "fused blocks walk their tiles XCD by XCD; bit 0: one-wave-per-tile launches, bit 1: group-split launches") \
    X(IRBW_FOLD,         "FFGPU_IRBW_FOLD",         INT,  0,             TUNING,  "k_irbw: never widen the reduction region to all G partial sums (folding rounds)") \
    X(IRB_ECH,           "FFGPU_IRB_ECH",           INT,  0,             TUNING,  "k_irb: expanded channels per chunk, 16 or 32 (0: by shape)") \
    X(IRB_RESIDENT,      "FFGPU_IRB_RESIDENT",      INT,  1,             TUNING,  "k_irb: every chunk's constants in LDS never (0) / where it costs no workgroup (1) / wherever they fit (2)") \
    X(IRB_TW,            "FFGPU_IRB_TW",            INT,  0,             TUNING,  "k_irb: tile width (0: the measured table, then the search)") \
    X(IRB_TH,            "FFGPU_IRB_TH",            INT,  0,             TUNING,  "k_irb: tile height for the search (0: any)") \
    X(IRB_NF,            "FFGPU_IRB_NF",            INT,  0,             TUNING,  "k_irb: frames per tile for the search, 1 / 2 / 4 (0: any)") \
    X(IRB_NOTABLE,       "FFGPU_IRB_NOTABLE",       INT,  0,             TUNING,  "k_irb: skip the measured table of tiles, search") \
    X(IRB_NW,            "FFGPU_IRB_NW",            INT,  8,             TUNING,  "k_irb: waves per workgroup, 8 or 4") \
    X(IRB_NOKS,          "FFGPU_IRB_NOKS",          INT,  0,             TUNING,  "k_irb: idle waves take no slices of the channel loop") \
    X(IRB_SKIP,          "FFGPU_IRB_SKIP",          INT,  0,             LAB,     "k_irb: ablation mask, 1 no input loads, 2 no expand, 4 no depthwise / project, 8 no stores (wrong results)") \
    X(IRB_TRACE,         "FFGPU_IRB_TRACE",         INT,  0,             LAB,     "lab builds with -DIRB_TRACE=1: every fused-block launch is followed by its in-kernel timeline on stderr") \
    X(VERBOSE_IRB,       "FFGPU_VERBOSE_IRB",       INT,  0,             LAB,     "print the plan line of every fused-block launch to stderr")

#ifdef FFGPU_DIAG
#define FFGPU_KNOBS_DIAG(X) \
    X(DBG_SKIP,          "FFGPU_DBG_SKIP",          TEXT, 0,             LAB,     "make DIAG=1: \"lo:hi\" drops the launches of layers lo .. hi (wrong results)") \
    X(DBG_KEEP,          "FFGPU_DBG_KEEP",          TEXT, 0,             LAB,     "make DIAG=1: \"lo:hi\" drops every launch but those of layers lo .. hi (wrong results)")
#else
#define FFGPU_KNOBS_DIAG(X)
#endif
#if defined(XT_TRACE) && XT_TRACE
#define FFGPU_KNOBS_XT(X) \
    X(PWXT_TRACE,        "FFGPU_PWXT_TRACE",        TEXT, 0,             LAB,     "builds with -DXT_TRACE=1: file that one traced k_pw_x3t launch dumps its per-tile timeline to")
#else
#define FFGPU_KNOBS_XT(X)
#endif
#define FFGPU_KNOBS(X) FFGPU_KNOBS_MAIN(X) FFGPU_KNOBS_DIAG(X) FFGPU_KNOBS_XT(X)

struct KnobRow { const char *name; KnobKind kind; int dflt; KnobClass cls; const char *text; };
#define X(id, name, kind, dflt, cls, text) K_##id,
enum Knob { FFGPU_KNOBS(X) K_COUNT, K_NONE = -1 };
#undef X
#define X(id, name, kind, dflt, cls, text) { name, KNOB_##kind, dflt, KNOB_##cls, text },
static constexpr KnobRow ffgpu_knob_rows[K_COUNT] = { FFGPU_KNOBS(X) };
#undef X

static inline int knob_int_(const KnobRow &r, int dflt) { const char *v = getenv(r.name); return v && *v ? atoi(v) : dflt; }
static inline int knob(Knob k)
{
    const KnobRow &r = ffgpu_knob_rows[k];
    assert((r.kind == KNOB_INT && r.dflt != KNOB_COMPUTED) || r.kind == KNOB_ON);
    if (r.kind == KNOB_INT) return knob_int_(r, r.dflt);
    const char *v = getenv(r.name);
    return v && atoi(v) != 0;
}
static inline int knob_or(Knob k, int dflt)
{
    const KnobRow &r = ffgpu_knob_rows[k];
    assert(r.kind == KNOB_INT && r.dflt == KNOB_COMPUTED);
    return knob_int_(r, dflt);
}
static inline bool knob_set(Knob k) { assert(ffgpu_knob_rows[k].kind == KNOB_SET); return getenv(ffgpu_knob_rows[k].name) != nullptr; }
static inline const char *knob_text(Knob k) { assert(ffgpu_knob_rows[k].kind == KNOB_TEXT); return getenv(ffgpu_knob_rows[k].name); }

static inline int ffgpu_knobs_lines(char *buf, size_t cap)
{
    static const char *const kinds[] = { "INT", "ON", "SET", "TEXT" }, *const classes[] = { "product", "tuning", "test", "lab" };
    size_t n = 0;
    if (cap) buf[0] = 0;
    for (int k = 0; k < K_COUNT; k++) {
        const KnobRow &r = ffgpu_knob_rows[k];
        const char *const env = getenv(r.name);
        char dflt[16] = "-", val[16];
        if (r.kind == KNOB_INT && r.dflt == KNOB_COMPUTED) snprintf(dflt, sizeof dflt, "computed");
        else if (r.kind != KNOB_TEXT) snprintf(dflt, sizeof dflt, "%d", r.dflt);
        if (r.kind == KNOB_TEXT) snprintf(val, sizeof val, env ? "set" : "unset");
        else if (r.kind == KNOB_SET) snprintf(val, sizeof val, "%d", (int)knob_set((Knob)k));
        else if (r.kind == KNOB_INT && r.dflt == KNOB_COMPUTED && !(env && *env)) snprintf(val, sizeof val, "default");
        else snprintf(val, sizeof val, "%d", r.kind == KNOB_INT && r.dflt == KNOB_COMPUTED ? knob_or((Knob)k, 0) : knob((Knob)k));
        n += (size_t)snprintf(n < cap ? buf + n : nullptr, n < cap ? cap - n : 0, "%s %s %s %s %s %s\n", r.name, kinds[r.kind], dflt, classes[r.cls], val, r.text);
    }
    return (int)n;
}
```

include/ffcnn_hip.h:

```cpp
#ifndef FFCNN_AMD_FFCNN_HIP_H
#define FFCNN_AMD_FFCNN_HIP_H

#include <stddef.h>
#include "ffcnn.h"

#ifdef __cplusplus
extern "C" {
#endif

#define FFGPU_MAX_DET   128



typedef struct {
    int  count;
    int  ncand;
    int  overflow;
    int  nfull;
    BBOX box[FFGPU_MAX_DET];
} ffgpu_frame_dets;

typedef struct ffgpu_exec ffgpu_exec;

#define FFGPU_KEEP_ALL   1
#define FFGPU_COMPAT_V6  2
#define FFGPU_NO_GRAPH   4
#define FFGPU_NO_FUSE    8
#define FFGPU_HOST_DETS  16
#define FFGPU_SPLIT2     32

#define FFGPU_CONCURRENT 64

#define FFGPU_BF16_PW   128

int         ffgpu_device_count(void);
int         ffgpu_set_device(int ordinal);
const char *ffgpu_last_error(void);
const char *ffgpu_build_info(void);

int ffgpu_net_weights_dev(NET *net, void **dev_ptr, size_t *bytes);
int ffgpu_net_weights_commit(NET *net, void *stream);

ffgpu_exec *ffgpu_exec_create(NET *net, int batch, int flags);
void        ffgpu_exec_destroy(ffgpu_exec *ex);
int         ffgpu_exec_batch(const ffgpu_exec *ex);
size_t      ffgpu_exec_arena_bytes(const ffgpu_exec *ex);
int         ffgpu_exec_kernel_count(const ffgpu_exec *ex);
int         ffgpu_exec_work_model(const ffgpu_exec *ex, double *hbm_bytes, double *flops);

int ffgpu_exec_set_scale(ffgpu_exec *ex, int s1, int s2);

int ffgpu_exec_forward_dev(ffgpu_exec *ex, const float *d_frames, void *stream);

int ffgpu_exec_forward_host(ffgpu_exec *ex, const float *h_frames);

int ffgpu_exec_forward_bgr_dev(ffgpu_exec *ex, const unsigned char *d_bgr, int w, int h,
                               const float mean[3], const float norm[3], void *stream);

typedef struct {
    const unsigned char *bgr;
    int w, h;
    int pitch;
    int reserved;
} ffgpu_bgr_frame;

int ffgpu_exec_forward_bgr_frames_dev(ffgpu_exec *ex, const ffgpu_bgr_frame *frames, int nframes,
                                      const float mean[3], const float norm[3], void *stream);

#define FFGPU_YUV_BT601_LIMITED 0
#define FFGPU_YUV_BT601_FULL    1
#define FFGPU_YUV_BT709_LIMITED 2
#define FFGPU_YUV_BT709_FULL    3

typedef struct {
    const unsigned char *y;
    const unsigned char *uv;
    int w, h;
    int pitch_y;
    int pitch_uv;
    int matrix;
    int reserved;
} ffgpu_nv12_frame;

int ffgpu_exec_forward_nv12_frames_dev(ffgpu_exec *ex, const ffgpu_nv12_frame *frames, int nframes,
                                       const float mean[3], const float norm[3], void *stream);

int ffgpu_exec_dets_dev(ffgpu_exec *ex, void **dev_ptr, size_t *bytes);
const ffgpu_frame_dets *ffgpu_exec_dets_host(ffgpu_exec *ex);
int ffgpu_exec_set_ring(ffgpu_exec *ex, void *dev_ring, int slots);
int ffgpu_exec_set_ring_strided(ffgpu_exec *ex, void *dev_ring, int slots, int slot_records);
int ffgpu_exec_read_dets(ffgpu_exec *ex, ffgpu_frame_dets *host_out, int max_frames);
int ffgpu_exec_read_boxes(ffgpu_exec *ex, int frame, BBOX *host_out, int cap);
int ffgpu_exec_cand_capacity(const ffgpu_exec *ex);
int ffgpu_exec_graph_captures(const ffgpu_exec *ex);

int ffgpu_exec_read_layer(ffgpu_exec *ex, int layer, int frame, float *host_out, size_t cap_floats);

int ffgpu_exec_hash_layers(ffgpu_exec *ex, unsigned long long *host_out, int cap);

int ffgpu_exec_profile(ffgpu_exec *ex, const float *d_frames, float us_by_kind[LAYER_TYPE_TOTOAL]);

int ffgpu_exec_profile_steps(ffgpu_exec *ex, const float *d_frames, int *layer_of, float *us, int cap);
int ffgpu_exec_step_model(const ffgpu_exec *ex, int *layer_of, double *hbm_bytes, int cap);

typedef struct ffgpu_node ffgpu_node;
#define FFGPU_NODE_LOOPBACK 1
#define FFGPU_NODE_DEPTH(n) (((n) & 0xf) << 8)

void        ffgpu_shard_range(int total, int rank, int world, int *lo, int *hi);
ffgpu_node *ffgpu_node_create(NET *net, int ndev, const int *devices, int global_batch, int exec_flags, int node_flags);
void        ffgpu_node_destroy(ffgpu_node *node);
int         ffgpu_node_ndev(const ffgpu_node *node);
int         ffgpu_node_shard(const ffgpu_node *node, int rank, int *lo, int *hi, int *device);
int         ffgpu_node_set_scale(ffgpu_node *node, int s1, int s2);
int         ffgpu_node_depth(const ffgpu_node *node);
int         ffgpu_node_rccl_ranks(const ffgpu_node *node);
float      *ffgpu_node_input_dev(ffgpu_node *node, int rank);
float      *ffgpu_node_input_slot_dev(ffgpu_node *node, int rank, int slot);
int         ffgpu_node_forward(ffgpu_node *node, ffgpu_frame_dets *host_out);
int         ffgpu_node_forward_host(ffgpu_node *node, const float *h_frames, ffgpu_frame_dets *host_out);
long        ffgpu_node_submit(ffgpu_node *node, const float *h_frames);
int         ffgpu_node_wait(ffgpu_node *node, long ticket, ffgpu_frame_dets *host_out);
int         ffgpu_node_run(ffgpu_node *node, long steps, ffgpu_frame_dets *host_out);

int ffgpu_groupconv_dev(const float *d_in, const float *d_filt, float *d_out, int batch,
                        int iw, int ih, int ic, int groups, int pad, int stride,
                        int fs, int fn, int ow, int oh, int oc, int act,
                        int flags, int variant, void *stream);

enum {
    FFGPU_K_AUTO = 0,
    FFGPU_K_GENERIC = 1,
    FFGPU_K_DW_STREAM = 2,
    FFGPU_K_DW_LDS = 3,
    FFGPU_K_PW_MFMA = 4,
    FFGPU_K_PW_GEMM = 5,
    FFGPU_K_DENSE_SMALL = 7,
    FFGPU_K_IGEMM = 8,
    FFGPU_K_PW_BF16 = 9,
    FFGPU_K_GROUP_THIN = 10,
    FFGPU_K_PW_X3 = 11,
    FFGPU_K_CONV_X3 = 12,
    FFGPU_K_PW_X3T = 13
};

const char *ffgpu_groupconv_kernel_name(int batch, int iw, int ih, int ic, int groups, int pad,
                                        int stride, int fs, int fn, int variant);

float ffgpu_groupconv_time_dev(const float *d_in, const float *d_filt, float *d_out, int batch,
                               int iw, int ih, int ic, int groups, int pad, int stride,
                               int fs, int fn, int ow, int oh, int oc, int act,
                               int flags, int variant, int warmup, int iters, void *stream);

float ffgpu_irb_dev(const float *d_in, const float *d_w1, const float *d_wd, const float *d_w2,
                    const float *d_res, float *d_out, int batch, int iw, int ih, int ic, int ec, int oc,
                    int stride, int act1, int actd, int act2, int res_act, int warmup, int iters, void *stream);

int ffgpu_irb_plan_text(int batch, int iw, int ih, int ic, int ec, int oc, int stride, int act1, int actd, int act2, int res_act,
                        int flags, char *buf, int cap);

int ffgpu_irb_stage_plan_text(int batch, int iw, int ih, int blocks, int act1, int actd, int flags, char *buf, int cap);

int ffgpu_front_plan_text(int batch, int pw, int ph, int form, char *buf, int cap);

int ffgpu_irb_instantiations(char *buf, int cap);

int ffgpu_knobs_text(char *buf, int cap);

float ffgpu_dwpw_dev(const float *d_in, const float *d_wd, const float *d_wp, float *d_out, int batch, int iw, int ih,
                     int c, int oc, int fs, int actd, int actp, int warmup, int iters, void *stream);

size_t ffgpu_packed_records_bytes(int batch, int cap);
int    ffgpu_unpack_records(const void *block, int batch, int cap, ffgpu_frame_dets *out);
int    ffgpu_pack_records(const void *d_records, int nslots, long slot_stride_records, int batch, int cap, void *d_out, void *stream);

typedef struct {
    int image;
    int x0, y0;
    int reserved;
} ffgpu_tile;

#define FFGPU_MERGE_LDS_SLOTS 1024

size_t ffgpu_merge_tiles_scratch_bytes(int ntiles, int list_stride);
int    ffgpu_merge_tiles_dev(const void *d_records, const void *d_lists, int list_stride, const ffgpu_tile *tiles, int ntiles, int nimages,
                             float thresh, int use_min, void *d_out_records, void *d_out_lists, void *d_scratch, size_t scratch_bytes, void *stream);

int ffgpu_exec_merge_tiles(ffgpu_exec *ex, const ffgpu_tile *tiles, int ntiles, int nimages, void *stream);
int ffgpu_exec_merged_dev(ffgpu_exec *ex, void **dev_ptr, size_t *bytes);
int ffgpu_exec_read_merged(ffgpu_exec *ex, ffgpu_frame_dets *host_out, int max_images);
int ffgpu_exec_read_merged_boxes(ffgpu_exec *ex, int image, BBOX *host_out, int cap);

typedef struct { int x0, y0, w, h; } ffgpu_tile_rect;
int ffgpu_tile_plan(int img_w, int img_h, int tile_w, int tile_h, int overlap_x, int overlap_y, int align, ffgpu_tile_rect *out, int cap);

typedef struct {
    unsigned char color[4];
    const unsigned char *palette;
    int npalette;
    int thickness;
} ffgpu_draw_style;

int ffgpu_draw_boxes_bgr_dev (const void *d_records, const void *d_lists, int list_stride, const int *list_first,
                              const ffgpu_bgr_frame  *targets, int ntargets, const ffgpu_draw_style *style, void *stream);
int ffgpu_draw_boxes_nv12_dev(const void *d_records, const void *d_lists, int list_stride, const int *list_first,
                              const ffgpu_nv12_frame *targets, int ntargets, const ffgpu_draw_style *style, void *stream);

#define FFGPU_DRAW_ENTRIES 0
#define FFGPU_DRAW_MERGED  1
int ffgpu_exec_draw_bgr (ffgpu_exec *ex, int which, const ffgpu_bgr_frame  *targets, int ntargets, const ffgpu_draw_style *style, void *stream);
int ffgpu_exec_draw_nv12(ffgpu_exec *ex, int which, const ffgpu_nv12_frame *targets, int ntargets, const ffgpu_draw_style *style, void *stream);

#define FFGPU_CROP_F32 0
#define FFGPU_CROP_U8  1
typedef struct {
    int   out_w, out_h;
    int   form;
    int   per_target;
    float min_score;
    int   nclasses;
    const unsigned char *classes;
    int   margin_num, margin_den;
    float mean[3], norm[3];
    int   reserved;
} ffgpu_crop_spec;
typedef struct {
    int   target, box, type;
    float score;
    int   x0, y0, w, h;
    int   sw, sh, s1, s2;
} ffgpu_crop;

size_t ffgpu_crop_table_bytes(int capacity);
size_t ffgpu_crop_slot_bytes(int out_w, int out_h, int form);

int ffgpu_crop_boxes_bgr_dev (const void *d_records, const void *d_lists, int list_stride, const int *list_first, const ffgpu_bgr_frame  *sources,
                              int ntargets, const ffgpu_crop_spec *spec, void *d_out, void *d_table, int capacity, void *stream);
int ffgpu_crop_boxes_nv12_dev(const void *d_records, const void *d_lists, int list_stride, const int *list_first, const ffgpu_nv12_frame *sources,
                              int ntargets, const ffgpu_crop_spec *spec, void *d_out, void *d_table, int capacity, void *stream);

#define FFGPU_CROP_ENTRIES 0
#define FFGPU_CROP_MERGED  1
int ffgpu_exec_crop_bgr (ffgpu_exec *ex, int which, const ffgpu_bgr_frame  *sources, int ntargets, const ffgpu_crop_spec *spec,
                         void *d_out, void *d_table, int capacity, void *stream);
int ffgpu_exec_crop_nv12(ffgpu_exec *ex, int which, const ffgpu_nv12_frame *sources, int ntargets, const ffgpu_crop_spec *spec,
                         void *d_out, void *d_table, int capacity, void *stream);

int ffgpu_crops_to_source_dev(const void *d_table, int capacity, const void *d_records, const void *d_lists, int list_stride,
                              void *d_out_records, void *d_out_lists, void *stream);

#define FFGPU_TRACK_DETS 128
typedef struct {
    int   capacity;
    int   max_missed;
    int   min_hits;
    float iou_thresh;
    float min_score;
    float birth_score;
    int   class_aware;
    int   reserved;
} ffgpu_track_spec;
typedef struct {
    int   id, type;
    float score, x1, y1, x2, y2;
    int   hits, missed;
    int   born, det;
    int   reserved;
} ffgpu_track;

size_t ffgpu_track_state_bytes(int nstreams, int capacity);
int ffgpu_track_reset_dev(void *d_state, int nstreams, int capacity, int which_stream, void *stream);

int ffgpu_track_boxes_dev(const void *d_records, const void *d_lists, int list_stride, const int *list_first, const int *streams, int ntargets,
                          const ffgpu_track_spec *spec, void *d_state, int nstreams, void *d_ids, void *d_out_records, void *d_out_lists, void *stream);

#define FFGPU_TRACK_ENTRIES 0
#define FFGPU_TRACK_MERGED  1
int ffgpu_exec_track(ffgpu_exec *ex, int which, const int *streams, int ntargets, const ffgpu_track_spec *spec, void *d_state, int nstreams,
                     void *d_ids, void *d_out_records, void *d_out_lists, void *stream);

#define FFGPU_FEAT_FLAT    0
#define FFGPU_FEAT_MEAN    1
#define FFGPU_FEAT_MAX     2
#define FFGPU_POST_NONE    0
#define FFGPU_POST_SOFTMAX 1
#define FFGPU_POST_L2      2
typedef struct {
    int layer;
    int pool, post;
    int reserved;
} ffgpu_feature_spec;

int ffgpu_feature_dim(int c, int h, int w, int pool);
int ffgpu_exec_feature_dim(const ffgpu_exec *ex, const ffgpu_feature_spec *spec);

int ffgpu_features_dev(const float *d_in, int n, int c, int h, int w, int pool, int post, float *d_out, long out_stride, void *stream);

int ffgpu_exec_features(ffgpu_exec *ex, const ffgpu_feature_spec *spec, float *d_out, long out_stride, void *stream);

#define FFGPU_TOPK_MAX 16
typedef struct { int index; float value; } ffgpu_label;
int ffgpu_topk_dev(const float *d_in, int n, int d, long in_stride, int k, void *d_out, void *stream);

#define FFGPU_RELABEL_KEEP_SCORE  0
#define FFGPU_RELABEL_LABEL_SCORE 1
typedef struct {
    float min_value;
    int   type_base;
    int   score_mode;
    int   reserved;
// ... 362 lines not shown
```

Measured before the change: 207,400.

## Pack two frames per wave in k_irb_thin for concurrent executors

Adds a paired form of the thin inverted-residual kernel in which one wave covers two frames, with 3, 4 or 5 output columns per lane instead of 4. This fills lanes that sit idle when a row uses fewer than 64 lanes. The paired form is used only when the executor runs with FFGPU_CONCURRENT, and a knob can switch it off. The change also adds a plan-text API and a flags variant of the irb test entry point. In exchange there is more edge handling (first-column masking, unaligned stores for 3 and 5 columns) and possibly higher register pressure.

```diff
diff --git a/ffcnn_amd/capi.py b/ffcnn_amd/capi.py
--- a/ffcnn_amd/capi.py
+++ b/ffcnn_amd/capi.py
@@ -274,7 +274,7 @@
            "ffgpu_exec_kernel_count", "ffgpu_exec_work_model", "ffgpu_exec_set_scale", "ffgpu_exec_forward_dev", "ffgpu_exec_forward_host",
            "ffgpu_exec_forward_bgr_dev", "ffgpu_exec_forward_bgr_frames_dev", "ffgpu_exec_forward_nv12_frames_dev", "ffgpu_exec_dets_dev", "ffgpu_exec_dets_host", "ffgpu_exec_set_ring", "ffgpu_exec_set_ring_strided", "ffgpu_exec_read_dets", "ffgpu_exec_read_layer", "ffgpu_exec_hash_layers",
            "ffgpu_exec_read_boxes", "ffgpu_exec_cand_capacity", "ffgpu_exec_graph_captures",
-           "ffgpu_exec_profile", "ffgpu_exec_profile_steps", "ffgpu_exec_step_model", "ffgpu_groupconv_dev", "ffgpu_groupconv_kernel_name", "ffgpu_groupconv_time_dev", "ffgpu_irb_dev", "ffgpu_irb_plan_text", "ffgpu_irb_stage_plan_text", "ffgpu_front_plan_text", "ffgpu_irb_instantiations", "ffgpu_knobs_text", "ffgpu_dwpw_dev", "ffgpu_packed_records_bytes", "ffgpu_pack_records", "ffgpu_unpack_records",
+           "ffgpu_exec_profile", "ffgpu_exec_profile_steps", "ffgpu_exec_step_model", "ffgpu_groupconv_dev", "ffgpu_groupconv_kernel_name", "ffgpu_groupconv_time_dev", "ffgpu_irb_dev", "ffgpu_irb_flags_dev", "ffgpu_irb_plan_text", "ffgpu_irb_thin_launch_text", "ffgpu_irb_stage_plan_text", "ffgpu_front_plan_text", "ffgpu_irb_instantiations", "ffgpu_knobs_text", "ffgpu_dwpw_dev", "ffgpu_packed_records_bytes", "ffgpu_pack_records", "ffgpu_unpack_records",
            "ffgpu_shard_range", "ffgpu_node_create", "ffgpu_node_destroy", "ffgpu_node_ndev", "ffgpu_node_shard", "ffgpu_node_set_scale",
            "ffgpu_node_input_dev", "ffgpu_node_input_slot_dev", "ffgpu_node_depth", "ffgpu_node_rccl_ranks", "ffgpu_node_forward", "ffgpu_node_forward_host",
            "ffgpu_node_submit", "ffgpu_node_wait", "ffgpu_node_run",
@@ -372,6 +372,9 @@
     L.ffgpu_groupconv_time_dev.argtypes = [vp, vp, vp] + [i] * 17 + [vp]
     L.ffgpu_irb_dev.restype = C.c_float
     L.ffgpu_irb_dev.argtypes = [vp] * 6 + [i] * 13 + [vp]
+    L.ffgpu_irb_flags_dev.restype = C.c_float
+    L.ffgpu_irb_flags_dev.argtypes = [vp] * 6 + [i] * 14 + [vp]
+    L.ffgpu_irb_thin_launch_text.argtypes = [i] * 12 + [C.c_char_p, i]
     L.ffgpu_irb_plan_text.argtypes = [i] * 12 + [C.c_char_p, i]
     L.ffgpu_irb_stage_plan_text.argtypes = [i] * 7 + [C.c_char_p, i]
     L.ffgpu_front_plan_text.argtypes = [i] * 4 + [C.c_char_p, i]
@@ -1688,10 +1691,17 @@
     return us
 
 
+def irb_thin_launch_text(shape, flags=0):
+    buf = C.create_string_buffer(256)
+    if lib().ffgpu_irb_thin_launch_text(*shape, flags, buf, len(buf)) < 0:
+        raise RuntimeError("ffgpu_irb_thin_launch_text failed: %s" % last_error())
+    return buf.value.decode()
+
+
 def irb_dev(d_in, d_w1, d_wd, d_w2, d_res, d_out, batch, iw, ih, ic, ec, oc, stride, act1=2, actd=2, act2=0, res_act=0,
-            warmup=0, iters=0, stream=None):
-    us = lib().ffgpu_irb_dev(d_in, d_w1, d_wd, d_w2, d_res, d_out, batch, iw, ih, ic, ec, oc, stride, act1, actd, act2, res_act,
-                             warmup, iters, stream)
+            warmup=0, iters=0, stream=None, flags=0):
+    us = lib().ffgpu_irb_flags_dev(d_in, d_w1, d_wd, d_w2, d_res, d_out, batch, iw, ih, ic, ec, oc, stride, act1, actd, act2, res_act, flags,
+                                   warmup, iters, stream)
     if us < 0:
         raise RuntimeError("ffgpu_irb_dev failed: %s" % last_error())
     return us
diff --git a/ffcnn_amd/csrc/ffgpu_conv_kernels.inc b/ffcnn_amd/csrc/ffgpu_conv_kernels.inc
--- a/ffcnn_amd/csrc/ffgpu_conv_kernels.inc
+++ b/ffcnn_amd/csrc/ffgpu_conv_kernels.inc
@@ -1019,17 +1019,65 @@
     return 0;
 }
 
+static constexpr bool thin_pair_built(int ic, int ncp) { return !(ic == 8 && ncp == 5); }
+static int thin_pair_ncp(int W, int ic)
+{
+    for (int nc = 3; nc <= 5; nc++)
+        if (W % nc == 0 && W / nc <= 32) return thin_pair_built(ic, nc) ? nc : 0;
+    return 0;
+}
+
+struct ThinForm { int ncp, band, nbands; long ntasks; int grid; };
+static ThinForm thin_form(const IrbDesc &d)
+{
+    ThinForm f;
+    const int ncp = thin_pair_ncp(d.W, d.ic);
+    const bool pair = ncp && d.N >= 2 && (d.flags & FFGPU_CONCURRENT) && knob(K_THIN_PAIR) != 0;
+    const int units = pair ? (d.N + 1) / 2 : d.N;
+    f.ncp = pair ? ncp : 0;
+    f.band = pair ? knob_or(K_THIN_BAND, thin_band(units, d.H)) : d.plan.band;
+    f.nbands = (d.H + f.band - 1) / f.band;
+    f.ntasks = (long)units * f.nbands;
+    f.grid = pair ? (int)((f.ntasks + 3) / 4) : d.plan.grid;
+    return f;
+}
+
+template <int IC, int EC, int OC>
+static int irb_thin_pair_launch(const ThinP &p, const ThinForm &f, hipStream_t s)
+{
+    if (f.ncp == 3) hipLaunchKernelGGL((k_irb_thin_pair<IC, EC, OC, 3>), dim3((unsigned)f.grid), dim3(256), 0, s, p);
+    else if (f.ncp == 4) hipLaunchKernelGGL((k_irb_thin_pair<IC, EC, OC, 4>), dim3((unsigned)f.grid), dim3(256), 0, s, p);
+    else if constexpr (thin_pair_built(IC, 5)) hipLaunchKernelGGL((k_irb_thin_pair<IC, EC, OC, 5>), dim3((unsigned)f.grid), dim3(256), 0, s, p);
+    else { ffgpu_set_error("irb_thin_pair: no instantiation for %d columns per lane of %d channels", f.ncp, IC); return -1; }
+    LAUNCH_OK("irb_thin_pair");
+    return 0;
+}
+
 typedef int (*IrbThinLaunch)(const ThinP &, const IrbPlan &, hipStream_t);
-struct IrbThinKernel { int IC, OC; IrbThinLaunch launch; };
-static const IrbThinKernel irb_thin_kernels[] = { { 8, 4, irb_thin_launch<8, 8, 4> }, { 4, 4, irb_thin_launch<4, 8, 4> }, { 8, 8, irb_thin_launch<8, 8, 8> }, { 4, 8, irb_thin_launch<4, 8, 8> } };
+typedef int (*IrbThinPairLaunch)(const ThinP &, const ThinForm &, hipStream_t);
+struct IrbThinKernel { int IC, OC; IrbThinLaunch launch; IrbThinPairLaunch pair; };
+static const IrbThinKernel irb_thin_kernels[] = { { 8, 4, irb_thin_launch<8, 8, 4>, irb_thin_pair_launch<8, 8, 4> }, { 4, 4, irb_thin_launch<4, 8, 4>, irb_thin_pair_launch<4, 8, 4> },
+                                                  { 8, 8, irb_thin_launch<8, 8, 8>, irb_thin_pair_launch<8, 8, 8> }, { 4, 8, irb_thin_launch<4, 8, 8>, irb_thin_pair_launch<4, 8, 8> } };
 
 static int launch_irb_thin(const IrbDesc &d, hipStream_t s)
 {
-    const ThinP p = thin_params(d);
+    ThinP p = thin_params(d);
+    const ThinForm f = thin_form(d);
+    if (f.ncp) { p.band = f.band; p.nbands = f.nbands; p.ntasks = f.ntasks; }
     for (const IrbThinKernel &k : irb_thin_kernels)
-        if (k.IC == d.ic && k.OC == d.oc) return k.launch(p, d.plan, s);
+        if (k.IC == d.ic && k.OC == d.oc) return f.ncp ? k.pair(p, f, s) : k.launch(p, d.plan, s);
     ffgpu_set_error("irb_thin: no instantiation for %d -> 8 -> %d channels", d.ic, d.oc);
     return -1;
+}
+
+int ffgpu_irb_thin_launch_line(const IrbDesc &d, char *buf, size_t cap)
+{
+    if (d.plan.family != IRB_THIN) return snprintf(buf, cap, "unsupported");
+    const ThinForm f = thin_form(d);
+    char key[48];
+    if (f.ncp) snprintf(key, sizeof key, "thin_pair<%d,8,%d,%d>", d.ic, d.oc, f.ncp);
+    else snprintf(key, sizeof key, "thin<%d,8,%d>", d.ic, d.oc);
+    return snprintf(buf, cap, "%s W=%d H=%d N=%d band=%d nbands=%d ntasks=%ld grid=%d block=256", key, d.W, d.H, d.N, f.band, f.nbands, f.ntasks, f.grid);
 }
 
 typedef int (*IrbwLaunch)(const IrbwP &, const IrbPlan &, hipStream_t);
diff --git a/ffcnn_amd/csrc/ffgpu_dev.hpp b/ffcnn_amd/csrc/ffgpu_dev.hpp
--- a/ffcnn_amd/csrc/ffgpu_dev.hpp
+++ b/ffcnn_amd/csrc/ffgpu_dev.hpp
@@ -72,6 +72,7 @@
 int    ffgpu_irb_pack(const IrbDesc &d, float *pk, hipStream_t s);
 int    ffgpu_launch_irb(const IrbDesc &d, hipStream_t s);
 int    ffgpu_irb_plan_line(const IrbDesc &d, char *buf, size_t cap);
+int    ffgpu_irb_thin_launch_line(const IrbDesc &d, char *buf, size_t cap);
 int    ffgpu_irb_keys(char *buf, size_t cap);
 #define IRBS_MAXB 8
 bool   ffgpu_irb_stage_ok(const IrbDesc *blocks, int B);
diff --git a/ffcnn_amd/csrc/ffgpu_exec.hip b/ffcnn_amd/csrc/ffgpu_exec.hip
--- a/ffcnn_amd/csrc/ffgpu_exec.hip
+++ b/ffcnn_amd/csrc/ffgpu_exec.hip
@@ -1840,14 +1840,32 @@
     return ffgpu_knobs_lines(buf, (size_t)cap);
 }
 
+extern "C" int ffgpu_irb_thin_launch_text(int batch, int iw, int ih, int ic, int ec, int oc, int stride, int act1, int actd, int act2, int res_act, int flags, char *buf, int cap)
+{
+    if (!buf || cap < 1 || batch < 1 || iw < 1 || ih < 1 || stride < 1) { ffgpu_set_error("irb_thin_launch_text: bad arguments"); return -1; }
+    IrbDesc d{};
+    irb_fill(d, batch, iw, ih, ic, ec, oc, stride, act1, actd, act2, res_act);
+    d.flags = flags & FFGPU_CONCURRENT;
+    (void)ffgpu_irb_plan(d);
+    return ffgpu_irb_thin_launch_line(d, buf, (size_t)cap);
+}
+
 extern "C" float ffgpu_irb_dev(const float *d_in, const float *d_w1, const float *d_wd, const float *d_w2,
                                const float *d_res, float *d_out, int batch, int iw, int ih, int ic, int ec, int oc,
                                int stride, int act1, int actd, int act2, int res_act, int warmup, int iters, void *stream)
+{
+    return ffgpu_irb_flags_dev(d_in, d_w1, d_wd, d_w2, d_res, d_out, batch, iw, ih, ic, ec, oc, stride, act1, actd, act2, res_act, 0, warmup, iters, stream);
+}
+
+extern "C" float ffgpu_irb_flags_dev(const float *d_in, const float *d_w1, const float *d_wd, const float *d_w2,
+                                     const float *d_res, float *d_out, int batch, int iw, int ih, int ic, int ec, int oc,
+                                     int stride, int act1, int actd, int act2, int res_act, int flags, int warmup, int iters, void *stream)
 {
     hipStream_t s = (hipStream_t)stream;
     IrbDesc d{};
     d.in = d_in; d.out = d_out; d.residual = d_res; d.w1 = d_w1; d.wd = d_wd; d.w2 = d_w2;
     irb_fill(d, batch, iw, ih, ic, ec, oc, stride, act1, actd, act2, res_act);
+    d.flags = flags & FFGPU_CONCURRENT;
     if (!d_in || !d_out || !d_w1 || !d_wd || !d_w2 || !ffgpu_irb_plan(d)) { ffgpu_set_error("irb_dev: unsupported block shape"); return -1.f; }
     float *pk = nullptr;
     if (hipMalloc(&pk, ffgpu_irb_pack_floats(d) * sizeof(float)) != hipSuccess) { ffgpu_set_error("irb_dev: hipMalloc failed"); return -1.f; }
diff --git a/ffcnn_amd/csrc/ffgpu_irb_thin.inc b/ffcnn_amd/csrc/ffgpu_irb_thin.inc
--- a/ffcnn_amd/csrc/ffgpu_irb_thin.inc
+++ b/ffcnn_amd/csrc/ffgpu_irb_thin.inc
@@ -12,181 +12,14 @@
 template <int IC, int EC, int OC>
 __global__ void __launch_bounds__(256) __attribute__((amdgpu_waves_per_eu(2))) k_irb_thin(ThinP p)
 {
-    static_assert(EC % 2 == 0 && OC % 2 == 0, "channel pairs");
-    constexpr int K4 = (IC + 3) & ~3, RL1 = K4 + 4, RL2 = ((EC + 3) & ~3) + 4, OCP = (OC + 3) & ~3, CP = EC / 2;
-    constexpr int T1 = (IC + 2) * 2, TD = 24, T2 = 2 * OCP;
-    __shared__ __attribute__((aligned(16))) float tw[CP * (T1 + TD + T2) + 2 * OCP];
-    float *t1 = tw, *td = tw + CP * T1, *t2 = td + CP * TD, *tsb = t2 + CP * T2;
-    for (int i = threadIdx.x; i < CP * T1; i += 256) {
-        const int cp = i / T1, j = (i % T1) >> 1, c = 2 * cp + (i & 1);
-        t1[i] = p.w1[c * RL1 + (j < IC ? j : K4 + (j - IC))];
-    }
-    for (int i = threadIdx.x; i < CP * TD; i += 256) {
-        const int cp = i / TD, j = (i % TD) >> 1, c = 2 * cp + (i & 1);
-        td[i] = j < 9 ? p.wd[c * 16 + j] : (j < 11 ? p.wd[c * 16 + 3 + j] : 0.f);
-    }
-    for (int i = threadIdx.x; i < CP * T2; i += 256) {
-        const int cp = i / T2, h = (i % T2) / OCP, k = i % OCP;
-        t2[i] = k < OC ? p.w2[k * RL2 + 2 * cp + h] : 0.f;
-    }
-    for (int i = threadIdx.x; i < 2 * OCP; i += 256) { const int k = i % OCP; tsb[i] = k < OC ? p.w2[k * RL2 + RL2 - 4 + i / OCP] : 0.f; }
-    __syncthreads();
-    const int lane = threadIdx.x & 63;
-    const int task = blockIdx.x * 4 + __builtin_amdgcn_readfirstlane(threadIdx.x >> 6);
-    if (task >= p.ntasks) return;
-    const int n = task / p.nbands, band_i = task - n * p.nbands;
-    const int lpr = p.W >> 2;
-    const bool on = lane < lpr, last_col = lane == lpr - 1;
-    const long HW = (long)p.W * p.H;
-    const unsigned cs = (unsigned)p.N * (unsigned)HW;
-    const unsigned lo = on ? lane * 4 : 0;
-    const float *ip = p.in + (long)n * HW;
-    float *op = p.out + (long)n * HW;
-    const float *rp = p.residual ? p.residual + (long)n * HW : nullptr;
-    const int y0 = band_i * p.band, y1 = min(y0 + p.band, p.H);
-    const v2f_t z2 = { 0.f, 0.f };
+    constexpr int NC = 4 + 0 * IC;
+    constexpr bool PAIR = IC < 0;
+#include "ffgpu_irb_thin_body.inc"
+}
 
-    auto load_row = [&](int r, v4f (&x)[IC]) {
-        const unsigned ro = (unsigned)min(max(r, 0), p.H - 1) * p.W + lo;
-#pragma unroll
-        for (int ci = 0; ci < IC; ci++) x[ci] = *reinterpret_cast<const v4f *>(ip + (ci * cs + ro));
-    };
-    struct W1T { v4f q[T1 / 4]; };
-    struct WDT { v4f q[TD / 4]; v4f w2[T2 / 4]; };
-    auto ld1 = [&](int cp) { W1T r;
-#pragma unroll
-        for (int j = 0; j < T1 / 4; j++) r.q[j] = *reinterpret_cast<const v4f *>(t1 + cp * T1 + 4 * j);
-        return r; };
-    auto ldd = [&](int cp) { WDT r;
-#pragma unroll
-        for (int j = 0; j < TD / 4; j++) r.q[j] = *reinterpret_cast<const v4f *>(td + cp * TD + 4 * j);
-#pragma unroll
-        for (int j = 0; j < T2 / 4; j++) r.w2[j] = *reinterpret_cast<const v4f *>(t2 + cp * T2 + 4 * j);
-        return r; };
-    auto pairof = [](const v4f (&q)[TD / 4 > T1 / 4 ? TD / 4 : T1 / 4], int j) { return (j & 1) ? (v2f_t){ q[j >> 1].z, q[j >> 1].w } : (v2f_t){ q[j >> 1].x, q[j >> 1].y }; };
-    (void)pairof;
-
-    v2f_t A[2][CP][4];
-    v4f X[2][IC];
-#pragma unroll
-    for (int c = 0; c < CP; c++)
-#pragma unroll
-        for (int j = 0; j < 4; j++) A[0][c][j] = A[1][c][j] = z2;
-    load_row(y0 - 1, X[0]);
-
-    auto step = [&](int r, auto PAR) {
-        constexpr int P = decltype(PAR)::value;
-        asm volatile("" ::: "memory");
-        const bool rin = r >= 0 && r < p.H, fin = r > y0;
-        const v4f (&x)[IC] = X[P];
-        v4f res[OC];
-        if (r < y1) load_row(r + 1, X[P ^ 1]);
-        if (fin && rp) {
-#pragma unroll
-            for (int k = 0; k < OC; k++) res[k] = *reinterpret_cast<const v4f *>(rp + (k * cs + (unsigned)(r - 1) * p.W + lo));
-        }
-        v2f_t o[OCP / 2][4];
-#pragma unroll
-        for (int k = 0; k < OCP / 2; k++)
-#pragma unroll
-            for (int j = 0; j < 4; j++) o[k][j] = z2;
-        W1T n1 = ld1(0);
-        __builtin_amdgcn_sched_barrier(0);
-#pragma unroll
-        for (int cp = 0; cp < CP; cp++) {
-            const W1T c1 = n1;
-            const WDT cd = ldd(cp);
-            __builtin_amdgcn_sched_barrier(0);
-            auto w1p = [&](int j) { return (j & 1) ? (v2f_t){ c1.q[j >> 1].z, c1.q[j >> 1].w } : (v2f_t){ c1.q[j >> 1].x, c1.q[j >> 1].y }; };
-            auto wdp = [&](int j) { return (j & 1) ? (v2f_t){ cd.q[j >> 1].z, cd.q[j >> 1].w } : (v2f_t){ cd.q[j >> 1].x, cd.q[j >> 1].y }; };
-            v2f_t win[6];
-            if (rin) {
-#pragma unroll
-                for (int j = 0; j < 4; j++) {
-                    v2f_t a = w1p(0) * x[0][j];
-#pragma unroll
-                    for (int ci = 1; ci < IC; ci++) a += w1p(ci) * x[ci][j];
-                    a = a * w1p(IC) + w1p(IC + 1);
-                    const v2f_t u = a * p.act1;
-                    win[1 + j] = (v2f_t){ act_max(a.x, u.x, act_floor(p.act1)), act_max(a.y, u.y, act_floor(p.act1)) };
-                }
-            } else {
-#pragma unroll
-                for (int j = 0; j < 4; j++) win[1 + j] = z2;
-            }
-            if (cp + 1 < CP) n1 = ld1(cp + 1);
-            win[0] = (v2f_t){ dpp_shr1(win[4].x), dpp_shr1(win[4].y) };
-            const v2f_t sr = { dpp_shl1(win[1].x), dpp_shl1(win[1].y) };
-            win[5] = (v2f_t){ last_col ? 0.f : sr.x, last_col ? 0.f : sr.y };
-            __builtin_amdgcn_sched_barrier(0);
-            if (fin) {
-#pragma unroll
-                for (int j = 0; j < 4; j++) {
-                    v2f_t d = A[P][cp][j];
-                    d += wdp(6) * win[j]; d += wdp(7) * win[j + 1]; d += wdp(8) * win[j + 2];
-                    d = d * wdp(9) + wdp(10);
-                    const v2f_t u = d * p.actd;
-                    d = (v2f_t){ act_max(d.x, u.x, act_floor(p.actd)), act_max(d.y, u.y, act_floor(p.actd)) };
-#pragma unroll
-                    for (int k = 0; k < OCP / 2; k++) {
-                        const v4f &wa = cd.w2[k >> 1], &wb = cd.w2[(OCP / 2 + k) >> 1];
-                        const v2f_t w2a = (k & 1) ? (v2f_t){ wa.z, wa.w } : (v2f_t){ wa.x, wa.y };
-                        const v2f_t w2b = ((OCP / 2 + k) & 1) ? (v2f_t){ wb.z, wb.w } : (v2f_t){ wb.x, wb.y };
-                        o[k][j] += w2a * d.x;
-                        o[k][j] += w2b * d.y;
-                    }
-                }
-            }
-#pragma unroll
-            for (int j = 0; j < 4; j++) {
-                v2f_t m = A[P ^ 1][cp][j];
-                m += wdp(3) * win[j]; m += wdp(4) * win[j + 1]; m += wdp(5) * win[j + 2];
-                A[P ^ 1][cp][j] = m;
-                v2f_t s = wdp(0) * win[j];
-                s += wdp(1) * win[j + 1]; s += wdp(2) * win[j + 2];
-                A[P][cp][j] = s;
-            }
-#pragma unroll
-            for (int j = 0; j < 4; j++) asm volatile("" : "+v"(A[0][cp][j]), "+v"(A[1][cp][j]));
-            if (fin) {
-#pragma unroll
-                for (int k = 0; k < OCP / 2; k++)
-#pragma unroll
-                    for (int j = 0; j < 4; j++) asm volatile("" : "+v"(o[k][j]));
-            }
-            __builtin_amdgcn_sched_barrier(0);
-        }
-        if (fin && on) {
-            v4f sb[2 * OCP / 4];
-#pragma unroll
-            for (int j = 0; j < 2 * OCP / 4; j++) sb[j] = *reinterpret_cast<const v4f *>(tsb + 4 * j);
-#pragma unroll
-            for (int k = 0; k < OC / 2; k++) {
-                const v4f &sq = sb[k >> 1], &bq = sb[(OCP / 2 + k) >> 1];
-                const v2f_t sc = (k & 1) ? (v2f_t){ sq.z, sq.w } : (v2f_t){ sq.x, sq.y };
-                const v2f_t bi = ((OCP / 2 + k) & 1) ? (v2f_t){ bq.z, bq.w } : (v2f_t){ bq.x, bq.y };
-                v2f_t v[4];
-#pragma unroll
-                for (int j = 0; j < 4; j++) {
-                    const v2f_t t = o[k][j] * sc + bi, u = t * p.act2;
-                    v[j] = (v2f_t){ act_max(t.x, u.x, act_floor(p.act2)), act_max(t.y, u.y, act_floor(p.act2)) };
-                }
-#pragma unroll
-                for (int h = 0; h < 2; h++) {
-                    v4f q = { v[0][h], v[1][h], v[2][h], v[3][h] };
-                    if (rp) {
-                        q += res[2 * k + h];
-                        q.x = act_max(q.x, p.res_act * q.x, act_floor(p.res_act)); q.y = act_max(q.y, p.res_act * q.y, act_floor(p.res_act)); q.z = act_max(q.z, p.res_act * q.z, act_floor(p.res_act)); q.w = act_max(q.w, p.res_act * q.w, act_floor(p.res_act));
-                    }
-                    *reinterpret_cast<v4f *>(op + ((2 * k + h) * cs + (unsigned)(r - 1) * p.W + lo)) = q;
-                }
-            }
-        }
-    };
-    int r = y0 - 1;
-    for (; r < y1; r += 2) {
-        step(r, std::integral_constant<int, 0>());
-        step(r + 1, std::integral_constant<int, 1>());
-    }
-    if (r == y1) step(r, std::integral_constant<int, 0>());
+template <int IC, int EC, int OC, int NC>
+__global__ void __launch_bounds__(256) __attribute__((amdgpu_waves_per_eu(2))) k_irb_thin_pair(ThinP p)
+{
+    constexpr bool PAIR = NC > 0;
+#include "ffgpu_irb_thin_body.inc"
 }
diff --git a/ffcnn_amd/csrc/ffgpu_irb_thin_body.inc b/ffcnn_amd/csrc/ffgpu_irb_thin_body.inc
--- /dev/null
+++ b/ffcnn_amd/csrc/ffgpu_irb_thin_body.inc
@@ -0,0 +1,205 @@
+    static_assert(EC % 2 == 0 && OC % 2 == 0, "channel pairs");
+    static_assert(PAIR ? (NC >= 3 && NC <= 5) : NC == 4, "columns per lane");
+    constexpr int K4 = (IC + 3) & ~3, RL1 = K4 + 4, RL2 = ((EC + 3) & ~3) + 4, OCP = (OC + 3) & ~3, CP = EC / 2;
+    constexpr int T1 = (IC + 2) * 2, TD = 24, T2 = 2 * OCP;
+    __shared__ __attribute__((aligned(16))) float tw[CP * (T1 + TD + T2) + 2 * OCP];
+    float *t1 = tw, *td = tw + CP * T1, *t2 = td + CP * TD, *tsb = t2 + CP * T2;
+    for (int i = threadIdx.x; i < CP * T1; i += 256) {
+        const int cp = i / T1, j = (i % T1) >> 1, c = 2 * cp + (i & 1);
+        t1[i] = p.w1[c * RL1 + (j < IC ? j : K4 + (j - IC))];
+    }
+    for (int i = threadIdx.x; i < CP * TD; i += 256) {
+        const int cp = i / TD, j = (i % TD) >> 1, c = 2 * cp + (i & 1);
+        td[i] = j < 9 ? p.wd[c * 16 + j] : (j < 11 ? p.wd[c * 16 + 3 + j] : 0.f);
+    }
+    for (int i = threadIdx.x; i < CP * T2; i += 256) {
+        const int cp = i / T2, h = (i % T2) / OCP, k = i % OCP;
+        t2[i] = k < OC ? p.w2[k * RL2 + 2 * cp + h] : 0.f;
+    }
+    for (int i = threadIdx.x; i < 2 * OCP; i += 256) { const int k = i % OCP; tsb[i] = k < OC ? p.w2[k * RL2 + RL2 - 4 + i / OCP] : 0.f; }
+    __syncthreads();
+    const int lane = threadIdx.x & 63;
+    const int task = blockIdx.x * 4 + __builtin_amdgcn_readfirstlane(threadIdx.x >> 6);
+    if (task >= p.ntasks) return;
+    const int n = task / p.nbands, band_i = task - n * p.nbands;
+    const int lpr = PAIR ? p.W / NC : p.W >> 2;
+    const int hl = PAIR ? lane & 31 : lane;
+    const bool have = !PAIR || lane < 32 || 2 * n + 1 < p.N;
+    const bool on = PAIR ? hl < lpr && have : lane < lpr, last_col = hl == lpr - 1, first_col = hl == 0;
+    const long HW = (long)p.W * p.H;
+    const unsigned cs = (unsigned)p.N * (unsigned)HW;
+    const unsigned lo = PAIR ? (hl < lpr ? hl * NC : 0) + (lane >= 32 && have ? (unsigned)HW : 0u) : (on ? lane * 4 : 0);
+    const float *ip = p.in + (long)(PAIR ? 2 * n : n) * HW;
+    float *op = p.out + (long)(PAIR ? 2 * n : n) * HW;
+    const float *rp = p.residual ? p.residual + (long)(PAIR ? 2 * n : n) * HW : nullptr;
+    const int y0 = band_i * p.band, y1 = min(y0 + p.band, p.H);
+    const v2f_t z2 = { 0.f, 0.f };
+
+    typedef float v4a4 __attribute__((ext_vector_type(4), aligned(4)));
+    typedef float v3a4 __attribute__((ext_vector_type(3), aligned(4)));
+    constexpr int NE = NC == 5 ? 1 : 0;
+    constexpr bool RES_LATE = PAIR && IC + OC + (NC == 5 ? 4 : 0) >= 16;
+    auto load_cols = [&](const float *src, v4f &q, float &e) __attribute__((always_inline)) {
+        if constexpr (NC == 4) q = *reinterpret_cast<const v4f *>(src);
+        else if constexpr (NC == 5) { q = (v4f)*reinterpret_cast<const v4a4 *>(src); e = src[4]; }
+        else { const v3a4 t = *reinterpret_cast<const v3a4 *>(src); q = (v4f){ t.x, t.y, t.z, 0.f }; }
+    };
+    auto load_row = [&](int r, v4f (&x)[IC], float (&xe)[IC * NE + 1]) {
+        const unsigned ro = (unsigned)min(max(r, 0), p.H - 1) * p.W + lo;
+#pragma unroll
+        for (int ci = 0; ci < IC; ci++) load_cols(ip + (ci * cs + ro), x[ci], xe[ci * NE]);
+    };
+    struct W1T { v4f q[T1 / 4]; };
+    struct WDT { v4f q[TD / 4]; v4f w2[T2 / 4]; };
+    auto ld1 = [&](int cp) { W1T r;
+#pragma unroll
+        for (int j = 0; j < T1 / 4; j++) r.q[j] = *reinterpret_cast<const v4f *>(t1 + cp * T1 + 4 * j);
+        return r; };
+    auto ldd = [&](int cp) { WDT r;
+#pragma unroll
+        for (int j = 0; j < TD / 4; j++) r.q[j] = *reinterpret_cast<const v4f *>(td + cp * TD + 4 * j);
+#pragma unroll
+        for (int j = 0; j < T2 / 4; j++) r.w2[j] = *reinterpret_cast<const v4f *>(t2 + cp * T2 + 4 * j);
+        return r; };
+    auto pairof = [](const v4f (&q)[TD / 4 > T1 / 4 ? TD / 4 : T1 / 4], int j) { return (j & 1) ? (v2f_t){ q[j >> 1].z, q[j >> 1].w } : (v2f_t){ q[j >> 1].x, q[j >> 1].y }; };
+    (void)pairof;
+
+    v2f_t A[2][CP][NC];
+    v4f X[2][IC];
+    float XE[2][IC * NE + 1];
+#pragma unroll
+    for (int c = 0; c < CP; c++)
+#pragma unroll
+        for (int j = 0; j < NC; j++) A[0][c][j] = A[1][c][j] = z2;
+    load_row(y0 - 1, X[0], XE[0]);
+
+    auto step = [&](int r, auto PAR) {
+        constexpr int P = decltype(PAR)::value;
+        asm volatile("" ::: "memory");
+        const bool rin = r >= 0 && r < p.H, fin = r > y0;
+        const v4f (&x)[IC] = X[P];
+        const float (&xe)[IC * NE + 1] = XE[P];
+        auto xcol = [&](int ci, int j) __attribute__((always_inline)) {
+            if constexpr (NC == 5) return j < 4 ? x[ci][j & 3] : xe[ci];
+            else return x[ci][j];
+        };
+        v4f res[OC];
+        float rese[OC * NE + 1];
+        if (r < y1) load_row(r + 1, X[P ^ 1], XE[P ^ 1]);
+        auto load_res = [&]() __attribute__((always_inline)) {
+#pragma unroll
+            for (int k = 0; k < OC; k++) load_cols(rp + (k * cs + (unsigned)(r - 1) * p.W + lo), res[k], rese[k * NE]);
+        };
+        if constexpr (!RES_LATE) if (fin && rp) load_res();
+        v2f_t o[OCP / 2][NC];
+#pragma unroll
+        for (int k = 0; k < OCP / 2; k++)
+#pragma unroll
+            for (int j = 0; j < NC; j++) o[k][j] = z2;
+        W1T n1 = ld1(0);
+        __builtin_amdgcn_sched_barrier(0);
+#pragma unroll
+        for (int cp = 0; cp < CP; cp++) {
+            const W1T c1 = n1;
+            const WDT cd = ldd(cp);
+            __builtin_amdgcn_sched_barrier(0);
+            auto w1p = [&](int j) { return (j & 1) ? (v2f_t){ c1.q[j >> 1].z, c1.q[j >> 1].w } : (v2f_t){ c1.q[j >> 1].x, c1.q[j >> 1].y }; };
+            auto wdp = [&](int j) { return (j & 1) ? (v2f_t){ cd.q[j >> 1].z, cd.q[j >> 1].w } : (v2f_t){ cd.q[j >> 1].x, cd.q[j >> 1].y }; };
+            v2f_t win[NC + 2];
+            if (rin) {
+#pragma unroll
+                for (int j = 0; j < NC; j++) {
+                    v2f_t a = w1p(0) * xcol(0, j);
+#pragma unroll
+                    for (int ci = 1; ci < IC; ci++) a += w1p(ci) * xcol(ci, j);
+                    a = a * w1p(IC) + w1p(IC + 1);
+                    const v2f_t u = a * p.act1;
+                    win[1 + j] = (v2f_t){ act_max(a.x, u.x, act_floor(p.act1)), act_max(a.y, u.y, act_floor(p.act1)) };
+                }
+            } else {
+#pragma unroll
+                for (int j = 0; j < NC; j++) win[1 + j] = z2;
+            }
+            if (cp + 1 < CP) n1 = ld1(cp + 1);
+            win[0] = (v2f_t){ dpp_shr1(win[NC].x), dpp_shr1(win[NC].y) };
+            if constexpr (PAIR) win[0] = (v2f_t){ first_col ? 0.f : win[0].x, first_col ? 0.f : win[0].y };
+            const v2f_t sr = { dpp_shl1(win[1].x), dpp_shl1(win[1].y) };
+            win[NC + 1] = (v2f_t){ last_col ? 0.f : sr.x, last_col ? 0.f : sr.y };
+            __builtin_amdgcn_sched_barrier(0);
+            if (fin) {
+#pragma unroll
+                for (int j = 0; j < NC; j++) {
+                    v2f_t d = A[P][cp][j];
+                    d += wdp(6) * win[j]; d += wdp(7) * win[j + 1]; d += wdp(8) * win[j + 2];
+                    d = d * wdp(9) + wdp(10);
+                    const v2f_t u = d * p.actd;
+                    d = (v2f_t){ act_max(d.x, u.x, act_floor(p.actd)), act_max(d.y, u.y, act_floor(p.actd)) };
+#pragma unroll
+                    for (int k = 0; k < OCP / 2; k++) {
+                        const v4f &wa = cd.w2[k >> 1], &wb = cd.w2[(OCP / 2 + k) >> 1];
+                        const v2f_t w2a = (k & 1) ? (v2f_t){ wa.z, wa.w } : (v2f_t){ wa.x, wa.y };
+                        const v2f_t w2b = ((OCP / 2 + k) & 1) ? (v2f_t){ wb.z, wb.w } : (v2f_t){ wb.x, wb.y };
+                        o[k][j] += w2a * d.x;
+                        o[k][j] += w2b * d.y;
+                    }
+                }
+            }
+#pragma unroll
+            for (int j = 0; j < NC; j++) {
+                v2f_t m = A[P ^ 1][cp][j];
+                m += wdp(3) * win[j]; m += wdp(4) * win[j + 1]; m += wdp(5) * win[j + 2];
+                A[P ^ 1][cp][j] = m;
+                v2f_t s = wdp(0) * win[j];
+                s += wdp(1) * win[j + 1]; s += wdp(2) * win[j + 2];
+                A[P][cp][j] = s;
+            }
+#pragma unroll
+            for (int j = 0; j < NC; j++) asm volatile("" : "+v"(A[0][cp][j]), "+v"(A[1][cp][j]));
+            if (fin) {
+#pragma unroll
+                for (int k = 0; k < OCP / 2; k++)
+#pragma unroll
+                    for (int j = 0; j < NC; j++) asm volatile("" : "+v"(o[k][j]));
+            }
+            __builtin_amdgcn_sched_barrier(0);
+        }
+        if (fin && on) {
+            if constexpr (RES_LATE) if (rp) load_res();
+            v4f sb[2 * OCP / 4];
+#pragma unroll
+            for (int j = 0; j < 2 * OCP / 4; j++) sb[j] = *reinterpret_cast<const v4f *>(tsb + 4 * j);
+#pragma unroll
+            for (int k = 0; k < OC / 2; k++) {
+                const v4f &sq = sb[k >> 1], &bq = sb[(OCP / 2 + k) >> 1];
+                const v2f_t sc = (k & 1) ? (v2f_t){ sq.z, sq.w } : (v2f_t){ sq.x, sq.y };
+                const v2f_t bi = ((OCP / 2 + k) & 1) ? (v2f_t){ bq.z, bq.w } : (v2f_t){ bq.x, bq.y };
+                v2f_t v[NC < 4 ? 4 : NC];
+#pragma unroll
+                for (int j = 0; j < NC; j++) {
+                    const v2f_t t = o[k][j] * sc + bi, u = t * p.act2;
+                    v[j] = (v2f_t){ act_max(t.x, u.x, act_floor(p.act2)), act_max(t.y, u.y, act_floor(p.act2)) };
+                }
+                if constexpr (NC < 4) v[3] = z2;
+#pragma unroll
+                for (int h = 0; h < 2; h++) {
+                    v4f q = { v[0][h], v[1][h], v[2][h], v[3][h] };
+                    float qe = NC == 5 ? v[NC - 1][h] : 0.f;
+                    if (rp) {
+                        q += res[2 * k + h];
+                        q.x = act_max(q.x, p.res_act * q.x, act_floor(p.res_act)); q.y = act_max(q.y, p.res_act * q.y, act_floor(p.res_act)); q.z = act_max(q.z, p.res_act * q.z, act_floor(p.res_act)); q.w = act_max(q.w, p.res_act * q.w, act_floor(p.res_act));
+                        if constexpr (NC == 5) { qe += rese[2 * k + h]; qe = act_max(qe, p.res_act * qe, act_floor(p.res_act)); }
+                    }
+                    float *dst = op + ((2 * k + h) * cs + (unsigned)(r - 1) * p.W + lo);
+                    if constexpr (NC == 4) *reinterpret_cast<v4f *>(dst) = q;
+                    else if constexpr (NC == 5) { *reinterpret_cast<v4a4 *>(dst) = (v4a4)q; dst[4] = qe; }
+                    else *reinterpret_cast<v3a4 *>(dst) = (v3a4){ q.x, q.y, q.z };
+                }
+            }
+        }
+    };
+    int r = y0 - 1;
+    for (; r < y1; r += 2) {
+        step(r, std::integral_constant<int, 0>());
+        step(r + 1, std::integral_constant<int, 1>());
+    }
+    if (r == y1) step(r, std::integral_constant<int, 0>());
diff --git a/ffcnn_amd/csrc/ffgpu_knobs.hpp b/ffcnn_amd/csrc/ffgpu_knobs.hpp
--- a/ffcnn_amd/csrc/ffgpu_knobs.hpp
+++ b/ffcnn_amd/csrc/ffgpu_knobs.hpp
@@ -77,7 +77,8 @@
      \
     X(NO_THIN,           "FFGPU_NO_THIN",           INT,  0,             PRODUCT, "8-channel blocks on the wave kernel instead of k_irb_thin") \
     X(THIN_BAND,         "FFGPU_THIN_BAND",         INT,  KNOB_COMPUTED, TUNING,  "k_irb_thin: rows per wave; default by batch and height (thin_band)") \
-    X(FRONT_BAND,        "FFGPU_FRONT_BAND",        INT,  KNOB_COMPUTED, TUNING,  "k_front: rows per wave; default as FFGPU_THIN_BAND") \
+    X(THIN_PAIR,         "FFGPU_THIN_PAIR",         INT,  1,             TUNING,  "k_irb_thin: 0 keeps FFGPU_CONCURRENT executors off the paired form (two frames per wave, 3 / 4 / 5 columns per lane); read at launch") \
+    X(FRONT_BAND,        "FFGPU_FRONT_BAND",       INT,  KNOB_COMPUTED, TUNING,  "k_front: rows per wave; default as FFGPU_THIN_BAND") \
     X(NO_FRONT,          "FFGPU_NO_FRONT",          INT,  0,             PRODUCT, "layers 0-3 as k_conv_first + k_irb_thin instead of k_front") \
     X(FRONT_MIN_PX,      "FFGPU_FRONT_MIN_PX",      INT,  262144,        TUNING,  "k_front: fewest output pixels of the batch") \
     X(FRONT_NC,          "FFGPU_FRONT_NC",          INT,  3,             PRODUCT, "k_front: output columns per lane, 3 where a row fits a wave that way, or 4") \
diff --git a/include/ffcnn_hip.h b/include/ffcnn_hip.h
--- a/include/ffcnn_hip.h
+++ b/include/ffcnn_hip.h
@@ -156,6 +156,13 @@
                     const float *d_res, float *d_out, int batch, int iw, int ih, int ic, int ec, int oc,
                     int stride, int act1, int actd, int act2, int res_act, int warmup, int iters, void *stream);
 
+float ffgpu_irb_flags_dev(const float *d_in, const float *d_w1, const float *d_wd, const float *d_w2,
+                          const float *d_res, float *d_out, int batch, int iw, int ih, int ic, int ec, int oc,
+                          int stride, int act1, int actd, int act2, int res_act, int flags, int warmup, int iters, void *stream);
+
+int ffgpu_irb_thin_launch_text(int batch, int iw, int ih, int ic, int ec, int oc, int stride, int act1, int actd, int act2, int res_act,
+                               int flags, char *buf, int cap);
+
 int ffgpu_irb_plan_text(int batch, int iw, int ih, int ic, int ec, int oc, int stride, int act1, int actd, int act2, int res_act,
                         int flags, char *buf, int cap);
 
```

Result: faster. 209,800 (median of 6 runs) (+1.2%).
